# nelaturuharsha/TurboPrune

Measured on NVIDIA H100. Metric: images_per_sec_resnet50_erk80_train_step, higher is better.
Workload: dtype bf16

## Files before the change

### include/turboprune_b200.h

```cpp
#ifndef TURBOPRUNE_B200_H
#define TURBOPRUNE_B200_H

#include <stddef.h>
#include <stdint.h>

#ifdef __cplusplus
extern "C" {
#endif

#define TP_OK                 0
#define TP_ERR_INVALID       -1
#define TP_ERR_WORKSPACE     -2
#define TP_ERR_CUDA          -3
#define TP_ERR_K_RANGE       -4
#define TP_ERR_UNSUPPORTED   -5
#define TP_ERR_DEVICE        -6

const char* tp_strerror(int code);
const char* tp_last_cuda_error(void);
int         tp_abi_version(void);
int         tp_device_sm_count(void);
int         tp_set_pdl(int on);

#define TP_SCORE_MAG      0
#define TP_SCORE_SNIP     1
#define TP_SCORE_SYNFLOW  2

size_t tp_topk_workspace_bytes(int n_seg, int64_t total_numel);
int tp_topk_threshold_mask(const void* const* w, const void* const* g, const void* const* m,
                           void* const* mask_out, const int64_t* numel, int n_seg,
                           int64_t k, int score_kind, float* thr_out,
                           void* ws, size_t ws_bytes, int64_t* info_out, void* stream);
int tp_topk_enqueue(const void* const* w, const void* const* g, const void* const* m,
                    void* const* mask_out, const int64_t* numel, int n_seg,
                    int64_t k, int score_kind, float* thr_out,
                    void* ws, size_t ws_bytes, int table_cached, void* stream);
int tp_topk_finish(const void* const* m, void* const* mask_out, const int64_t* numel, int n_seg,
                   int64_t k, int score_kind, float* thr_out,
                   void* ws, size_t ws_bytes, int64_t* info_out, void* stream);

int tp_apply_threshold(const void* const* w, const void* const* g, const void* const* m,
                       void* const* mask_out, const int64_t* numel, int n_seg,
                       int score_kind, const float* thr, void* ws, size_t ws_bytes, void* stream);

int tp_count_zeros(const void* const* m, const int64_t* numel, int n_seg,
                   int64_t* zeros_out, void* ws, size_t ws_bytes, void* stream);

int tp_stage_weights(const void* w, const void* mask, int cout, int cin, int r, int s,
                     void* wf, int cin_p, int wf_ld, void* wd, int cout_p, int cin_p2,
                     void* kmask_f, void* kmask_d, void* stream);
size_t tp_kblock_mask_words(int64_t columns);

typedef struct tp_stage_item {
  const void* w; const void* mask;
  void* wf; void* wd;
  int32_t cout, cin, r, s, cin_p, cout_p, wf_ld;
  void* kmask_f; void* kmask_d;
} tp_stage_item;
size_t tp_stage_batched_workspace_bytes(int n_items);
int tp_stage_weights_batched(const tp_stage_item* items, int n_items, int table_cached, void* kmask_all, size_t kmask_bytes,
                             void* ws, size_t ws_bytes, void* stream);

int tp_to_nhwc_bf16(const void* src, int src_dtype, int64_t sn, int64_t sc, int64_t sh, int64_t sw,
                    int n, int c, int h, int w, void* dst, int c_pad, void* stream);

int tp_im2col_c8(const void* x, int n, int h, int w, int r, int s, int stride_h, int stride_w,
                 int pad_h, int pad_w, int p, int q, void* xcol, int kp, void* stream);

int tp_im2col_stem(const void* src, int src_dtype, int64_t sn, int64_t sc, int64_t sh, int64_t sw,
                   int n, int c, int h, int w, int r, int s, int cg, int stride_h, int stride_w, int pad_h, int pad_w,
                   int p, int q, void* xcol, int kp, void* stream);

int tp_cifar_augment(const void* src, void* out, const int64_t* idx, const int64_t* shifts, const uint8_t* flip,
                     const int64_t* cut_y, const int64_t* cut_x, int cut_size,
                     int n, int c, int h, int w, int r, void* stream);
typedef struct tp_crop_entry {
  const void* src;
  int32_t H, W;
  int32_t top, left, h, w;
  int32_t flip;
  int32_t reserved;
} tp_crop_entry;
int tp_resized_crop(const tp_crop_entry* table, int n, int size, const float* mean255, const float* std255, void* out,
                    void* stream);
int tp_synth_normal(void* out, int64_t numel, uint64_t seed, uint64_t counter_offset, int raw_words, void* stream);
int tp_synth_labels(void* out, int64_t numel, int num_classes, uint64_t seed, uint64_t counter_offset, void* stream);

typedef struct tp_conv_desc {
  int32_t n, h, w, cin;
  int32_t cout, r, s;
  int32_t stride_h, stride_w, pad_h, pad_w;
  int32_t p, q;
} tp_conv_desc;

size_t tp_conv_workspace_bytes(const tp_conv_desc* d, int op);

int tp_conv_fprop(const tp_conv_desc* d, const void* x, const void* wf, const void* bias_f32,
                  void* y, void* ws, size_t ws_bytes, void* stream);
size_t tp_conv_stats_rows(const tp_conv_desc* d);
int tp_conv_fprop_stats(const tp_conv_desc* d, const void* x, const void* wf, const void* kmask_f, const void* bias_f32,
                        void* y, void* stats, void* ws, size_t ws_bytes, void* stream);
int tp_conv_dgrad(const tp_conv_desc* d, const void* dy, const void* wd, const void* kmask_d, const void* addend,
                  void* dx, void* ws, size_t ws_bytes, void* stream);
size_t tp_conv_dgrad_partial_rows(const tp_conv_desc* d);
int tp_conv_dgrad_bnrelu(const tp_conv_desc* d, const void* dy, const void* wd, const void* kmask_d,
                         const void* bn_y, const void* bn_weight, const void* bn_bias, const void* bn_mean, const void* bn_invstd,
                         void* g, void* partial, void* stream);
int tp_conv_wgrad(const tp_conv_desc* d, const void* x, const void* dy, const void* mask, const void* kmask_f,
                  int cin_real, void* dw, void* db, void* ws, size_t ws_bytes, void* stream);

int tp_bn_forward_ext(const void* y, const void* residual, void* z, int64_t M, int C,
                      const void* weight, const void* bias, void* running_mean, void* running_var,
                      void* num_batches_tracked, float momentum, float eps, int training, int relu,
                      void* save_mean, void* save_invstd, const void* ext_stats, int64_t ext_rows,
                      void* ws, size_t ws_bytes, void* stream);

size_t tp_bn_workspace_bytes(int64_t m, int c);
int tp_bn_forward(const void* y, const void* residual, void* z, int64_t m, int c,
                  const void* weight, const void* bias, void* running_mean, void* running_var,
                  void* num_batches_tracked, float momentum, float eps, int training, int relu,
                  void* save_mean, void* save_invstd, void* ws, size_t ws_bytes, void* stream);
int tp_bn_backward(const void* dz, const void* z, const void* y, int64_t m, int c, const void* weight, const void* bias,
                   const void* save_mean, const void* save_invstd, int relu, void* dy, void* dres,
                   void* dweight, void* dbias, void* ws, size_t ws_bytes, void* stream);

int tp_bn_backward_ext(const void* g, const void* y, int64_t M, int C, const void* weight, const void* bias,
                       const void* save_mean, const void* save_invstd, const void* partial_rows, int64_t n_rows,
                       void* dy, void* dweight, void* dbias, void* ws, size_t ws_bytes, void* stream);
int tp_maxpool_forward(const void* x, void* y, void* idx, int n, int h, int w, int c, int k, int stride, int pad,
                       int p, int q, void* stream);
int tp_maxpool_backward(const void* dy, const void* idx, void* dx, int n, int h, int w, int c, int k, int stride, int pad,
                        int p, int q, void* stream);

int tp_sgd_momentum(void* const* w, const void* const* g, void* const* buf, const int64_t* numel,
                    int n_seg, const float* lr_dev, float momentum, float weight_decay,
                    int first_step, int table_cached, void* ws, size_t ws_bytes, void* stream);
size_t tp_segtable_workspace_bytes(int n_seg);

int tp_p2p_allreduce_mask(void* const* peer_bufs, void* const* signal_pads, int rank, int world,
                          int64_t numel, const void* mask, float scale, void* out,
                          int algo, int timeout_ms, int* status_dev, void* stream);

int tp_p2p_allreduce_nvls(void* const* peer_bufs, void* const* signal_pads, void* multicast_buf, int rank, int world,
                          int64_t numel, const void* mask, float scale, void* out,
                          int timeout_ms, int* status_dev, void* stream);

#ifdef __cplusplus
}
#endif
#endif
```

### turboprune_b200/_cabi.py

```python
import ctypes
import os
from ctypes import POINTER, c_char_p, c_float, c_int, c_int32, c_int64, c_size_t, c_uint64, c_void_p

from . import build as _build

TP_SCORE_MAG, TP_SCORE_SNIP, TP_SCORE_SYNFLOW = 0, 1, 2
TP_ERR_K_RANGE = -4

_lib = None


class ConvDesc(ctypes.Structure):
    _fields_ = [(n, c_int32) for n in
                ("n", "h", "w", "cin", "cout", "r", "s", "stride_h", "stride_w", "pad_h", "pad_w", "p", "q")]


class StageItem(ctypes.Structure):
    _fields_ = [("w", c_void_p), ("mask", c_void_p), ("wf", c_void_p), ("wd", c_void_p)] + \
               [(n, c_int32) for n in ("cout", "cin", "r", "s", "cin_p", "cout_p", "wf_ld")] + \
               [("kmask_f", c_void_p), ("kmask_d", c_void_p)]


class CropEntry(ctypes.Structure):
    _fields_ = [("src", c_void_p)] + [(n, c_int32) for n in ("H", "W", "top", "left", "h", "w", "flip", "reserved")]


SIGNATURES = {
    "tp_strerror": (c_char_p, [c_int]),
    "tp_last_cuda_error": (c_char_p, []),
    "tp_abi_version": (c_int, []),
    "tp_device_sm_count": (c_int, []),
    "tp_set_pdl": (c_int, [c_int]),
    "tp_topk_workspace_bytes": (c_size_t, [c_int, c_int64]),
    "tp_topk_threshold_mask": (c_int, [POINTER(c_void_p), POINTER(c_void_p), POINTER(c_void_p), POINTER(c_void_p),
                                       POINTER(c_int64), c_int, c_int64, c_int, c_void_p, c_void_p, c_size_t,
                                       POINTER(c_int64), c_void_p]),
    "tp_topk_enqueue": (c_int, [POINTER(c_void_p), POINTER(c_void_p), POINTER(c_void_p), POINTER(c_void_p),
                                POINTER(c_int64), c_int, c_int64, c_int, c_void_p, c_void_p, c_size_t, c_int, c_void_p]),
    "tp_topk_finish": (c_int, [POINTER(c_void_p), POINTER(c_void_p), POINTER(c_int64), c_int, c_int64, c_int, c_void_p,
                               c_void_p, c_size_t, POINTER(c_int64), c_void_p]),
    "tp_apply_threshold": (c_int, [POINTER(c_void_p), POINTER(c_void_p), POINTER(c_void_p), POINTER(c_void_p),
                                   POINTER(c_int64), c_int, c_int, c_void_p, c_void_p, c_size_t, c_void_p]),
    "tp_count_zeros": (c_int, [POINTER(c_void_p), POINTER(c_int64), c_int, c_void_p, c_void_p, c_size_t, c_void_p]),
    "tp_stage_weights": (c_int, [c_void_p, c_void_p, c_int, c_int, c_int, c_int, c_void_p, c_int, c_int, c_void_p, c_int,
                                 c_int, c_void_p, c_void_p, c_void_p]),
    "tp_kblock_mask_words": (c_size_t, [c_int64]),
    "tp_stage_batched_workspace_bytes": (c_size_t, [c_int]),
    "tp_stage_weights_batched": (c_int, [POINTER(StageItem), c_int, c_int, c_void_p, c_size_t, c_void_p, c_size_t, c_void_p]),
    "tp_to_nhwc_bf16": (c_int, [c_void_p, c_int, c_int64, c_int64, c_int64, c_int64, c_int, c_int, c_int, c_int,
                                c_void_p, c_int, c_void_p]),
    "tp_im2col_c8": (c_int, [c_void_p] + [c_int] * 11 + [c_void_p, c_int, c_void_p]),
    "tp_im2col_stem": (c_int, [c_void_p, c_int, c_int64, c_int64, c_int64, c_int64] + [c_int] * 13 + [c_void_p, c_int, c_void_p]),
    "tp_cifar_augment": (c_int, [c_void_p, c_void_p, c_void_p, c_void_p, c_void_p, c_void_p, c_void_p, c_int, c_int, c_int, c_int, c_int, c_int, c_void_p]),
    "tp_resized_crop": (c_int, [c_void_p, c_int, c_int, POINTER(c_float), POINTER(c_float), c_void_p, c_void_p]),
    "tp_synth_normal": (c_int, [c_void_p, c_int64, c_uint64, c_uint64, c_int, c_void_p]),
    "tp_synth_labels": (c_int, [c_void_p, c_int64, c_int, c_uint64, c_uint64, c_void_p]),
    "tp_conv_workspace_bytes": (c_size_t, [POINTER(ConvDesc), c_int]),
    "tp_conv_fprop": (c_int, [POINTER(ConvDesc), c_void_p, c_void_p, c_void_p, c_void_p, c_void_p, c_size_t, c_void_p]),
    "tp_conv_stats_rows": (c_size_t, [POINTER(ConvDesc)]),
    "tp_conv_fprop_stats": (c_int, [POINTER(ConvDesc), c_void_p, c_void_p, c_void_p, c_void_p, c_void_p, c_void_p, c_void_p, c_size_t, c_void_p]),
    "tp_conv_dgrad": (c_int, [POINTER(ConvDesc), c_void_p, c_void_p, c_void_p, c_void_p, c_void_p, c_void_p, c_size_t, c_void_p]),
    "tp_conv_dgrad_partial_rows": (c_size_t, [POINTER(ConvDesc)]),
    "tp_conv_dgrad_bnrelu": (c_int, [POINTER(ConvDesc), c_void_p, c_void_p, c_void_p, c_void_p, c_void_p, c_void_p, c_void_p, c_void_p,
                                     c_void_p, c_void_p, c_void_p]),
    "tp_bn_backward_ext": (c_int, [c_void_p, c_void_p, c_int64, c_int, c_void_p, c_void_p, c_void_p, c_void_p, c_void_p, c_int64,
                                   c_void_p, c_void_p, c_void_p, c_void_p, c_size_t, c_void_p]),
    "tp_conv_wgrad": (c_int, [POINTER(ConvDesc), c_void_p, c_void_p, c_void_p, c_void_p, c_int, c_void_p, c_void_p, c_void_p,
                              c_size_t, c_void_p]),
    "tp_sgd_momentum": (c_int, [POINTER(c_void_p), POINTER(c_void_p), POINTER(c_void_p), POINTER(c_int64), c_int,
                                c_void_p, c_float, c_float, c_int, c_int, c_void_p, c_size_t, c_void_p]),
    "tp_segtable_workspace_bytes": (c_size_t, [c_int]),
    "tp_p2p_allreduce_mask": (c_int, [POINTER(c_void_p), POINTER(c_void_p), c_int, c_int, c_int64, c_void_p, c_float,
                                      c_void_p, c_int, c_int, c_void_p, c_void_p]),
    "tp_bn_workspace_bytes": (c_size_t, [c_int64, c_int]),
    "tp_bn_forward": (c_int, [c_void_p, c_void_p, c_void_p, c_int64, c_int, c_void_p, c_void_p, c_void_p, c_void_p, c_void_p,
                              c_float, c_float, c_int, c_int, c_void_p, c_void_p, c_void_p, c_size_t, c_void_p]),
    "tp_bn_forward_ext": (c_int, [c_void_p, c_void_p, c_void_p, c_int64, c_int, c_void_p, c_void_p, c_void_p, c_void_p, c_void_p,
                                  c_float, c_float, c_int, c_int, c_void_p, c_void_p, c_void_p, c_int64, c_void_p, c_size_t, c_void_p]),
    "tp_bn_backward": (c_int, [c_void_p, c_void_p, c_void_p, c_int64, c_int, c_void_p, c_void_p, c_void_p, c_void_p, c_int, c_void_p,
                               c_void_p, c_void_p, c_void_p, c_void_p, c_size_t, c_void_p]),
    "tp_maxpool_forward": (c_int, [c_void_p, c_void_p, c_void_p] + [c_int] * 9 + [c_void_p]),
    "tp_maxpool_backward": (c_int, [c_void_p, c_void_p, c_void_p] + [c_int] * 9 + [c_void_p]),
    "tp_p2p_allreduce_nvls": (c_int, [POINTER(c_void_p), POINTER(c_void_p), c_void_p, c_int, c_int, c_int64, c_void_p, c_float,
                                      c_void_p, c_int, c_void_p, c_void_p]),
}


def lib_path() -> str:
    return _build.lib_path()


def load(build_if_missing: bool = False):
    global _lib
    if _lib is not None:
        return _lib
    path = lib_path()
    if not os.path.isfile(path):
        if build_if_missing:
            _build.build()
        else:
            raise RuntimeError(
                f"turboprune_b200: CUDA library not built ({path} missing). "
                "Run `python -c 'import __graft_entry__ as g; g.build()'`; there is no CPU fallback.")
    lib = ctypes.CDLL(path)
    for name, (res, args) in SIGNATURES.items():
        fn = getattr(lib, name)
        fn.restype = res
        fn.argtypes = args
    _lib = lib
    return lib


class TurboPruneError(RuntimeError):
    def __init__(self, code, where):
        lib = load()
        msg = lib.tp_strerror(code).decode()
        detail = lib.tp_last_cuda_error().decode() if code == -3 else ""
        super().__init__(f"{where}: {msg} (code {code}) {detail}".strip())
        self.code = code


def check(code: int, where: str):
    if code != 0:
        raise TurboPruneError(code, where)


def ptr_array(tensors):
    if tensors is None:
        return None
    arr = (c_void_p * len(tensors))()
    for i, t in enumerate(tensors):
        arr[i] = t.data_ptr() if t is not None else None
    return arr


def i64_array(vals):
    arr = (c_int64 * len(vals))()
    for i, v in enumerate(vals):
        arr[i] = int(v)
    return arr


def stream_ptr(device=None):
    import torch
    return c_void_p(torch.cuda.current_stream(device).cuda_stream)
```

### turboprune_b200/csrc/tp_common.cuh

```cuda
#pragma once
#include <cuda_runtime.h>
#include <cuda_bf16.h>
#include <stdint.h>
#include <stdio.h>
#include "../../include/turboprune_b200.h"

namespace tp {

void set_last_cuda_error(cudaError_t e, const char* where);

#define TP_CUDA_CHECK(expr)                                             \
  do {                                                                  \
    cudaError_t _e = (expr);                                            \
    if (_e != cudaSuccess) {                                            \
      ::tp::set_last_cuda_error(_e, #expr);                             \
      return TP_ERR_CUDA;                                               \
    }                                                                   \
  } while (0)

#define TP_LAUNCH_CHECK() TP_CUDA_CHECK(cudaGetLastError())

int sm_count();
int bind_device_of(const void* p);
inline size_t align_up(size_t x, size_t a) { return (x + a - 1) / a * a; }

bool pdl_enabled();
#ifdef __CUDACC__
__device__ __forceinline__ void pdl_wait() { asm volatile("griddepcontrol.wait;" ::: "memory"); }
__device__ __forceinline__ void pdl_trigger() { asm volatile("griddepcontrol.launch_dependents;" ::: "memory"); }
__device__ __forceinline__ void pdl_enter() { pdl_trigger(); pdl_wait(); }

template <typename... KA, typename... A>
inline cudaError_t launch(void (*kernel)(KA...), dim3 grid, dim3 block, size_t smem, cudaStream_t st, A&&... args) {
  cudaLaunchConfig_t cfg = {};
  cfg.gridDim = grid; cfg.blockDim = block; cfg.dynamicSmemBytes = smem; cfg.stream = st;
  cudaLaunchAttribute attr[1];
  attr[0].id = cudaLaunchAttributeProgrammaticStreamSerialization;
  attr[0].val.programmaticStreamSerializationAllowed = 1;
  cfg.attrs = attr; cfg.numAttrs = pdl_enabled() ? 1 : 0;
  return cudaLaunchKernelEx(&cfg, kernel, static_cast<KA>(args)...);
}
#endif

struct Arena {
  char* base; size_t cap; size_t off;
  Arena(void* p, size_t bytes) : base((char*)p), cap(bytes), off(0) {}
  void* take(size_t bytes, size_t align = 256) {
    size_t o = align_up(off, align);
    if (o + bytes > cap) return nullptr;
    off = o + bytes;
    return base + o;
  }
};

struct Seg {
  const float* w;
  const float* g;
  const float* m;
  float*       mo;
  float*       buf;
  long long    n;
  long long    start;
  long long    tile0;
};

constexpr int kTileElems = 4096;

int upload_segs(Arena& ar, const void* const* w, const void* const* g, const void* const* m,
                void* const* mo, void* const* buf, const int64_t* numel, int n_seg,
                Seg** dev_out, long long* tiles_out, long long* total_out, cudaStream_t st);

__device__ __forceinline__ int find_seg(const Seg* __restrict__ segs, int n_seg, long long tile) {
  int lo = 0, hi = n_seg - 1;
  while (lo < hi) {
    int mid = (lo + hi + 1) >> 1;
    if (segs[mid].tile0 <= tile) lo = mid; else hi = mid - 1;
  }
  return lo;
}
__device__ __forceinline__ int find_seg_by_elem(const Seg* __restrict__ segs, int n_seg, long long e) {
  int lo = 0, hi = n_seg - 1;
  while (lo < hi) {
    int mid = (lo + hi + 1) >> 1;
    if (segs[mid].start <= e) lo = mid; else hi = mid - 1;
  }
  return lo;
}

__device__ __forceinline__ float4 ld_stream(const float4* p) {
  float4 r;
  asm volatile("ld.global.nc.L1::no_allocate.v4.f32 {%0,%1,%2,%3}, [%4];"
               : "=f"(r.x), "=f"(r.y), "=f"(r.z), "=f"(r.w) : "l"(p));
  return r;
}
__device__ __forceinline__ void st_stream(float4* p, float4 v) {
  asm volatile("st.global.L1::no_allocate.v4.f32 [%0], {%1,%2,%3,%4};"
               :: "l"(p), "f"(v.x), "f"(v.y), "f"(v.z), "f"(v.w) : "memory");
}

}
```

### turboprune_b200/csrc/tp_core.cu

```cuda
#include "tp_common.cuh"
#include <stdlib.h>
#include <string.h>
#include <vector>

namespace tp {

static thread_local char g_last_err[512] = "";

void set_last_cuda_error(cudaError_t e, const char* where) {
  snprintf(g_last_err, sizeof(g_last_err), "%s: %s (%s)", where, cudaGetErrorName(e), cudaGetErrorString(e));
}

static int g_pdl = -1;
bool pdl_enabled() {
  if (g_pdl < 0) { const char* e = getenv("TP_PDL"); g_pdl = (e && e[0] == '1') ? 1 : 0; }
  return g_pdl == 1;
}

int sm_count() {
  static int cached[64] = {0};
  int dev = 0;
  if (cudaGetDevice(&dev) != cudaSuccess || dev < 0 || dev >= 64) return 132;
  if (cached[dev] == 0) {
    int n = 0;
    if (cudaDeviceGetAttribute(&n, cudaDevAttrMultiProcessorCount, dev) != cudaSuccess || n <= 0) n = 132;
    cached[dev] = n;
  }
  return cached[dev];
}

typedef int (*PFN_cuCtxGetCurrent)(void**);
static PFN_cuCtxGetCurrent g_ctx_get_current = nullptr;

int bind_device_of(const void* p) {
  if (!p) return TP_OK;
  static bool looked_up = false;
  if (!looked_up) {
    void* fn = nullptr; cudaDriverEntryPointQueryResult q;
    if (cudaGetDriverEntryPoint("cuCtxGetCurrent", &fn, cudaEnableDefault, &q) == cudaSuccess) g_ctx_get_current = (PFN_cuCtxGetCurrent)fn;
    looked_up = true;
  }
  if (g_ctx_get_current) {
    void* ctx = nullptr;
    if (g_ctx_get_current(&ctx) == 0 && ctx != nullptr) return TP_OK;
  }
  cudaPointerAttributes a;
  if (cudaPointerGetAttributes(&a, p) != cudaSuccess) { cudaGetLastError(); return TP_OK; }
  if (a.type == cudaMemoryTypeDevice || a.type == cudaMemoryTypeManaged) {
    TP_CUDA_CHECK(cudaSetDevice(a.device));
  }
  return TP_OK;
}

int upload_segs(Arena& ar, const void* const* w, const void* const* g, const void* const* m,
                void* const* mo, void* const* buf, const int64_t* numel, int n_seg,
                Seg** dev_out, long long* tiles_out, long long* total_out, cudaStream_t st) {
  if (n_seg <= 0 || !numel) return TP_ERR_INVALID;
  std::vector<Seg> h(n_seg);
  long long start = 0, tile = 0;
  for (int i = 0; i < n_seg; ++i) {
    if (numel[i] < 0) return TP_ERR_INVALID;
    h[i].w = w ? (const float*)w[i] : nullptr;
    h[i].g = g ? (const float*)g[i] : nullptr;
    h[i].m = m ? (const float*)m[i] : nullptr;
    h[i].mo = mo ? (float*)mo[i] : nullptr;
    h[i].buf = buf ? (float*)buf[i] : nullptr;
    h[i].n = numel[i];
    h[i].start = start;
    h[i].tile0 = tile;
    start += numel[i];
    tile += (numel[i] + kTileElems - 1) / kTileElems;
  }
  Seg* d = (Seg*)ar.take(sizeof(Seg) * n_seg);
  if (!d) return TP_ERR_WORKSPACE;
  TP_CUDA_CHECK(cudaMemcpyAsync(d, h.data(), sizeof(Seg) * n_seg, cudaMemcpyHostToDevice, st));
  *dev_out = d;
  if (tiles_out) *tiles_out = tile;
  if (total_out) *total_out = start;
  return TP_OK;
}

}

extern "C" {

const char* tp_strerror(int code) {
  switch (code) {
    case TP_OK: return "ok";
    case TP_ERR_INVALID: return "invalid argument";
    case TP_ERR_WORKSPACE: return "workspace too small";
    case TP_ERR_CUDA: return "CUDA error (see tp_last_cuda_error)";
    case TP_ERR_K_RANGE: return "kthvalue(): selected number k out of range";
    case TP_ERR_UNSUPPORTED: return "unsupported configuration";
    case TP_ERR_DEVICE: return "device is not sm_90 (H100)";
    default: return "unknown error";
  }
}

const char* tp_last_cuda_error(void) { return tp::g_last_err; }
int tp_abi_version(void) { return 10; }
int tp_device_sm_count(void) { return tp::sm_count(); }
int tp_set_pdl(int on) { const int prev = tp::pdl_enabled() ? 1 : 0; tp::g_pdl = on ? 1 : 0; return prev; }

size_t tp_segtable_workspace_bytes(int n_seg) {
  return tp::align_up(sizeof(tp::Seg) * (size_t)(n_seg > 0 ? n_seg : 1), 256) + 256;
}

}
```

### turboprune_b200/csrc/tp_igemm.cu

```cuda
#include "tp_common.cuh"
#include "tp_ptx.cuh"
#include <cuda.h>
#include <mutex>

namespace tp {
using namespace ptx;

constexpr int kBlockM = 128;
constexpr int kBlockK = 64;
constexpr int kConsumers = 256;
constexpr int kThreads = kConsumers + 32;
constexpr int kProducerWarp = kConsumers / 32;
constexpr int kFwdThreads = 3 * 128;
constexpr int kMaxTaps = 64;

constexpr int kFwdProducerRegs = 56, kFwdConsumerRegs = 224;
static_assert(kFwdProducerRegs * 128 + kFwdConsumerRegs * 256 <= 168 * kFwdThreads, "fwd register split");

__host__ __device__ constexpr int fwd_stages(int block_n) { return block_n == 128 ? 5 : 8; }
__host__ __device__ constexpr int fwd_stg_bytes(int block_n) { return kBlockM * block_n * 2; }
__host__ __device__ constexpr int fwd_smem(int block_n) {
  return fwd_stages(block_n) * (kBlockM * kBlockK * 2 + block_n * kBlockK * 2) + 2 * fwd_stg_bytes(block_n) + 1024 + 512;
}

struct TapEntry { uint16_t off_w, off_h; int32_t kofs; };

constexpr int kMaxCls = 4;

struct ClsEntry {
  int M;
  int P_it, Q_it;
  int ntaps, tap0;
  int base_w, base_h;
  int oah, oaw;
  int tile0, m_groups;
};

struct FwdParams {
  int M, N;
  int ncls;
  ClsEntry cls[kMaxCls];
  int cchunks;
  int a_mode;
  int step_w, step_h;
  long long out_img_pix;
  int out_row_pix;
  int osh, osw;
  int linear;
  int ldc;
  int staged_store;
  __nv_bfloat16* out;
  const float* bias;
  const __nv_bfloat16* addend;
  float* stats;
  const __nv_bfloat16* bn_y;
  const float* bn_weight; const float* bn_bias; const float* bn_mean; const float* bn_invstd;
  const uint32_t* kmask;
  int kmask_words;
  TapEntry taps[kMaxTaps];
};

__device__ __forceinline__ const uint32_t* live_kmask(const uint32_t* km, int words, int N) {
  if (km && __ldg(km + (size_t)((N + 63) >> 6) * words) == 0u) return nullptr;
  return km;
}

struct KSkip {
  const uint32_t* base; int words, g0, g1; int cur_w; uint32_t bits;
  __device__ __forceinline__ void begin(const uint32_t* km, int wds, int n0, int block_n, int N) {
    base = km; words = wds; cur_w = -1; bits = 0u;
    g0 = n0 >> 6; g1 = min((min(n0 + block_n, N) + 63) >> 6, ((N + 63) >> 6));
  }
  __device__ __forceinline__ bool on(int kb) {
    const int wi = kb >> 5;
    if (wi != cur_w) {
      cur_w = wi; bits = 0u;
      if (wi < words) for (int g = g0; g < g1; ++g) bits |= __ldg(base + (size_t)g * words + wi);
      else bits = 0xffffffffu;
    }
    return (bits >> (kb & 31)) & 1u;
  }
  __device__ __forceinline__ bool take(int kb, bool last, bool any) { return on(kb) || (last && !any); }
};

struct WgParams {
  int Mc;
  int Kpix;
  int P_it, Q_it;
  int chunks, cchunks;
  int nb;
  int b_mode;
  int base_w, base_h, step_w, step_h;
  int m_tiles, n_tiles, splits, kb_per_split, kblocks;
  float* partial;
  const uint32_t* kmask;
  int kmask_words;
  TapEntry taps[kMaxTaps];
};

struct WgItem {
  int split, tile, m_t, n_t, chunk0, nvalid, kb0, kb1;
  __device__ __forceinline__ void set_tile(int m, int n, int m_tiles, int nb, int chunks) {
    m_t = m; n_t = n; tile = n * m_tiles + m;
    chunk0 = n * nb; nvalid = min(nb, chunks - chunk0);
  }
  __device__ __forceinline__ bool empty(const uint32_t* __restrict__ km, int words, int Mc) const {
    const int row_groups = (Mc + 63) >> 6;
    for (int r = 2 * m_t; r < 2 * m_t + 2 && r < row_groups; ++r)
      for (int c = chunk0; c < chunk0 + nvalid; ++c)
        if ((__ldg(km + (size_t)r * words + (c >> 5)) >> (c & 31)) & 1u) return false;
    return true;
  }
};

__device__ __forceinline__ WgItem wg_item(const WgParams& p, int nb, int item) {
  WgItem w;
  const int ntile = p.m_tiles * p.n_tiles;
  w.split = item / ntile;
  const int tile = item - w.split * ntile, n_t = tile / p.m_tiles;
  w.set_tile(tile - n_t * p.m_tiles, n_t, p.m_tiles, nb, p.chunks);
  w.kb0 = w.split * p.kb_per_split; w.kb1 = min(p.kblocks, w.kb0 + p.kb_per_split);
  return w;
}

__device__ __forceinline__ void decompose_pixel(int m, int P, int Q, int& n, int& p, int& q) {
  q = m % Q; int t = m / Q; p = t % P; n = t / P;
}

struct AMaps { CUtensorMap m[kMaxCls]; };

__device__ __forceinline__ void decode_tile(const FwdParams& p, int tile, int n_tiles, int& c, int& m_g, int& n_t) {
  c = 0;
#pragma unroll
  for (int j = 1; j < kMaxCls; ++j) if (j < p.ncls && tile >= p.cls[j].tile0) c = j;
  const int local = tile - p.cls[c].tile0;
  m_g = local / n_tiles; n_t = local - m_g * n_tiles;
}

template <int BLOCK_N>
__device__ __forceinline__ void fwd_mma_block(float (&acc)[BLOCK_N], uint32_t a_addr, uint32_t b_addr, uint32_t accumulate) {
  const uint64_t adesc = make_smem_desc(a_addr, 16, 1024);
  const uint64_t adesc_hi = make_smem_desc(a_addr + 64 * kBlockK * 2, 16, 1024);
  const uint64_t bdesc = make_smem_desc(b_addr, 16, 1024);
#pragma unroll
  for (int k = 0; k < kBlockK / 16; ++k) {
    if constexpr (BLOCK_N == 128) {
      wgmma_m64n128<0, 0>(acc, adesc + (uint64_t)(2 * k), bdesc + (uint64_t)(2 * k), accumulate | (uint32_t)k);
      wgmma_m64n128<0, 0>(acc + BLOCK_N / 2, adesc_hi + (uint64_t)(2 * k), bdesc + (uint64_t)(2 * k), accumulate | (uint32_t)k);
    } else {
      wgmma_m64n64<0, 0>(acc, adesc + (uint64_t)(2 * k), bdesc + (uint64_t)(2 * k), accumulate | (uint32_t)k);
      wgmma_m64n64<0, 0>(acc + BLOCK_N / 2, adesc_hi + (uint64_t)(2 * k), bdesc + (uint64_t)(2 * k), accumulate | (uint32_t)k);
    }
  }
}

template <int BLOCK_N, bool MULTI, bool BNB>
__global__ void __launch_bounds__(kFwdThreads, 1)
k_igemm_fwd(const __grid_constant__ AMaps tmA, const __grid_constant__ CUtensorMap tmB,
            const __grid_constant__ FwdParams p) {
  static_assert(BLOCK_N == 64 || BLOCK_N == 128, "wgmma N of the fwd kernel");
  static_assert(!BNB || !MULTI, "BatchNorm-backward epilogue: single class");
  constexpr int kABytes = kBlockM * kBlockK * 2;
  constexpr int kBBytes = BLOCK_N * kBlockK * 2;
  constexpr int kStageBytes = kABytes + kBBytes;
  constexpr int kStages = fwd_stages(BLOCK_N);
  extern __shared__ __align__(1024) uint8_t smem_raw[];
  uint8_t* smem = (uint8_t*)(((uintptr_t)smem_raw + 1023) & ~(uintptr_t)1023);
  pdl_trigger();
  constexpr int kStgBytes = fwd_stg_bytes(BLOCK_N);
  constexpr int kChunkStg = kBlockM * 64 * 2;
  uint8_t* const stg_base = smem + kStages * kStageBytes;
  uint64_t* full_bar = (uint64_t*)(stg_base + 2 * kStgBytes);
  uint64_t* empty_bar = full_bar + kStages;
  uint64_t* order_bar = empty_bar + kStages;
  int* ring_pos = (int*)(order_bar + 2);

  const int warp = threadIdx.x >> 5, lane = threadIdx.x & 31;
  const int n_tiles = (p.N + BLOCK_N - 1) / BLOCK_N;
  const int total_tiles = p.cls[p.ncls - 1].tile0 + p.cls[p.ncls - 1].m_groups * n_tiles;
  const int my_items = total_tiles > (int)blockIdx.x ? (total_tiles - (int)blockIdx.x + (int)gridDim.x - 1) / (int)gridDim.x : 0;
  auto get_tile = [&](int w, int& ci, int& m_g, int& n_t) {
    ci = 0;
    const int tile = (int)blockIdx.x + w * (int)gridDim.x;
    if (MULTI) decode_tile(p, tile, n_tiles, ci, m_g, n_t);
    else { m_g = tile / n_tiles; n_t = tile - m_g * n_tiles; }
  };

  if (threadIdx.x == 0) {
    for (int j = 0; j < p.ncls; ++j) prefetch_tmap(&tmA.m[j]);
    prefetch_tmap(&tmB);
    for (int i = 0; i < kStages; ++i) { mbar_init(&full_bar[i], 1); mbar_init(&empty_bar[i], 1); }
    mbar_init(&order_bar[0], 1); mbar_init(&order_bar[1], 1);
    fence_mbar_init();
  }
  __syncthreads();
  pdl_wait();

  if (warp < 4) {
    setmaxnreg_dec<kFwdProducerRegs>();
    if (threadIdx.x == 0) {
      int stage = 0; uint32_t phase = 0;
      const uint32_t* const km = live_kmask(p.kmask, p.kmask_words, p.N);
      for (int w = 0; w < my_items; ++w) {
        int ci, m_g, n_t; get_tile(w, ci, m_g, n_t);
        const ClsEntry& ce = p.cls[MULTI ? ci : 0];
        const CUtensorMap* const mapA = &tmA.m[MULTI ? ci : 0];
        const int m0 = m_g * kBlockM;
        int cn = 0, cp = 0, cq = 0;
        if (p.a_mode == 1) decompose_pixel(m0, ce.P_it, ce.Q_it, cn, cp, cq);
        const int cw = ce.base_w + cq * p.step_w, ch = ce.base_h + cp * p.step_h;
        auto load_block = [&](const TapEntry& te, int cc) {
          mbar_wait(&empty_bar[stage], phase ^ 1);
          uint8_t* sA = smem + stage * kStageBytes;
          uint8_t* sB = sA + kABytes;
          mbar_arrive_expect_tx(&full_bar[stage], kStageBytes);
          if (p.a_mode == 1)
            tma_load_im2col_4d(sA, mapA, &full_bar[stage], cc * kBlockK, cw, ch, cn, te.off_w, te.off_h);
          else
            tma_load_2d(sA, mapA, &full_bar[stage], te.kofs + cc * kBlockK, m0);
          tma_load_2d(sB, &tmB, &full_bar[stage], te.kofs + cc * kBlockK, n_t * BLOCK_N);
          if (++stage == kStages) { stage = 0; phase ^= 1; }
        };
        const int tap_base = MULTI ? ce.tap0 : 0;
        if (!km) {
          for (int tap = 0; tap < ce.ntaps; ++tap) {
            const TapEntry te = p.taps[tap_base + tap];
            for (int cc = 0; cc < p.cchunks; ++cc) load_block(te, cc);
          }
        } else {
          KSkip ks; bool any = false;
          ks.begin(km, p.kmask_words, n_t * BLOCK_N, BLOCK_N, p.N);
          for (int tap = 0; tap < ce.ntaps; ++tap) {
            const TapEntry te = p.taps[tap_base + tap];
            for (int cc = 0; cc < p.cchunks; ++cc) {
              const bool last = tap == ce.ntaps - 1 && cc == p.cchunks - 1;
              if (!ks.take((te.kofs >> 6) + cc, last, any)) continue;
              any = true;
              load_block(te, cc);
            }
          }
        }
      }
    }
  } else {
    setmaxnreg_inc<kFwdConsumerRegs>();
    const int cw = (warp >> 2) - 1;
    const int q = warp & 3;
    const int wtid = threadIdx.x & 127;
    const int bar_id = 1 + cw;
    const uint32_t* const km = live_kmask(p.kmask, p.kmask_words, p.N);
    const uint32_t stg = smem_u32(stg_base + cw * kStgBytes);
    const int fr0 = q * 16 + (lane >> 2);
    const uint32_t fsw = (uint32_t)(lane >> 2);
    const uint32_t frag_base = stg + (uint32_t)(fr0 * 128 + (lane & 3) * 4);
    const int r_in = lane >> 3, c16 = lane & 7;
    const uint32_t buf = stg + (uint32_t)(q * 32 * 128);
    const uint32_t rd_even = buf + r_in * 128 + ((uint32_t)(c16 ^ r_in) << 4);
    const uint32_t rd_odd = buf + (r_in + 4) * 128 + ((uint32_t)(c16 ^ (r_in + 4)) << 4);
    for (int it = 0, w = cw; w < my_items; ++it, w += 2) {
      int ci, m_g, n_t; get_tile(w, ci, m_g, n_t);
      const ClsEntry& ce = p.cls[MULTI ? ci : 0];
      const bool has_acc = MULTI ? ce.ntaps > 0 : true;
      const int m_t = m_g;

      int stage = 0; uint32_t phase = 0;
      const int turn = it + cw;
      if (turn > 0) {
        mbar_wait(&order_bar[cw], (uint32_t)((turn - 1) & 1));
        const int pos = *(volatile int*)ring_pos;
        stage = pos >> 1; phase = (uint32_t)(pos & 1);
      }
      bar_sync(bar_id, 128);
      auto pass_turn = [&]() {
        if (wtid == 0) { *(volatile int*)ring_pos = stage * 2 + (int)phase; mbar_arrive(&order_bar[cw ^ 1]); }
      };
      float acc[BLOCK_N];
      if (has_acc) {
#pragma unroll
        for (int i = 0; i < BLOCK_N; ++i) acc[i] = 0.f;
        int prev = -1;
        auto mma_block = [&](uint32_t accumulate) {
          mbar_wait(&full_bar[stage], phase);
          const uint32_t s_addr = smem_u32(smem + stage * kStageBytes);
          wgmma_fence();
          fwd_mma_block<BLOCK_N>(acc, s_addr, s_addr + kABytes, accumulate);
          wgmma_commit();
          wgmma_wait<1>();
          if (prev >= 0 && wtid == 0) mbar_arrive(&empty_bar[prev]);
          prev = stage;
          if (++stage == kStages) { stage = 0; phase ^= 1; }
        };
        KSkip ks; uint32_t any = 0;
        if (km) ks.begin(km, p.kmask_words, n_t * BLOCK_N, BLOCK_N, p.N);
        for (int tap = 0; tap < ce.ntaps; ++tap) {
          const int kb0 = p.taps[(MULTI ? ce.tap0 : 0) + tap].kofs >> 6;
          for (int cc = 0; cc < p.cchunks; ++cc) {
            const bool last = tap == ce.ntaps - 1 && cc == p.cchunks - 1;
            if (km && !ks.take(kb0 + cc, last, any)) continue;
            mma_block(any);
            any = 1;
          }
        }
        pass_turn();
        wgmma_wait<0>();
        acc_fence(acc);
        if (prev >= 0 && wtid == 0) mbar_arrive(&empty_bar[prev]);
      } else {
        pass_turn();
      }

      const long long wrow0 = (long long)m_t * kBlockM + q * 32;
      const int rows_left = (int)(ce.M - wrow0 < 32 ? (ce.M - wrow0 < 0 ? 0 : ce.M - wrow0) : 32);
      const long long ldc = p.ldc;
      const int N = p.N;
      long long ooff[MULTI ? 8 : 1];
      const long long rbase = (wrow0 + r_in) * ldc + c16 * 8;
      if (MULTI && p.staged_store) {
        int n, pp, qq; decompose_pixel((int)(wrow0 + r_in), ce.P_it, ce.Q_it, n, pp, qq);
#pragma unroll
        for (int i = 0; i < 8; ++i) {
          const long long px = (long long)n * p.out_img_pix + (long long)(pp * p.osh + ce.oah) * p.out_row_pix + (qq * p.osw + ce.oaw);
          ooff[i] = px * ldc + c16 * 8;
          qq += 4;
          while (qq >= ce.Q_it) { qq -= ce.Q_it; if (++pp == ce.P_it) { pp = 0; ++n; } }
        }
      }
      auto row_off = [&](int i) -> long long { return MULTI ? ooff[MULTI ? i : 0] : rbase + (long long)(i * 4) * ldc; };
      if (MULTI && !has_acc) {
        if (p.staged_store) {
#pragma unroll 1
          for (int c = 0; c < BLOCK_N; c += 64) {
            const int n0 = n_t * BLOCK_N + c;
            if (n0 >= N) break;
            if (n0 + c16 * 8 + 8 > N) continue;
            uint4 z[8];
#pragma unroll
            for (int i = 0; i < 8; ++i) {
              z[i] = make_uint4(0u, 0u, 0u, 0u);
              if (p.addend && i * 4 + r_in < rows_left) z[i] = *reinterpret_cast<const uint4*>(p.addend + row_off(i) + n0);
            }
#pragma unroll
            for (int i = 0; i < 8; ++i)
              if (i * 4 + r_in < rows_left) *reinterpret_cast<uint4*>(p.out + row_off(i) + n0) = z[i];
          }
        } else {
          const int row = m_t * kBlockM + wtid;
          if (row < ce.M) {
            int n, pp, qq; decompose_pixel(row, ce.P_it, ce.Q_it, n, pp, qq);
            const long long opix = (long long)n * p.out_img_pix + (long long)(pp * p.osh + ce.oah) * p.out_row_pix + (qq * p.osw + ce.oaw);
            for (int j = n_t * BLOCK_N; j < min(p.N, (n_t + 1) * BLOCK_N); ++j)
              p.out[opix * p.ldc + j] = p.addend ? p.addend[opix * p.ldc + j] : __float2bfloat16_rn(0.f);
          }
        }
        continue;
      }
      if (p.staged_store) {
        __nv_bfloat16* const gout = p.out;
        const __nv_bfloat16* const gadd = p.addend;
        const float* bias = p.bias;
        float* stats = p.stats ? p.stats + (long long)(m_t * 4 + q) * 2 * N + c16 * 8 : nullptr;
        if (gadd) {
          __syncwarp();
#pragma unroll
          for (int ch = 0; ch < BLOCK_N / 64; ++ch) {
            const int n0 = n_t * BLOCK_N + ch * 64;
            if (n0 >= N) break;
            const bool col_ok = n0 + c16 * 8 + 8 <= N;
            uint4 a[8];
#pragma unroll
            for (int i = 0; i < 8; ++i) {
              a[i] = make_uint4(0u, 0u, 0u, 0u);
              if (i * 4 + r_in < rows_left && col_ok) a[i] = *reinterpret_cast<const uint4*>(gadd + row_off(i) + n0);
            }
#pragma unroll
            for (int i = 0; i < 8; ++i) sts128(((i & 1) ? rd_odd : rd_even) + (uint32_t)(ch * kChunkStg + (i >> 1) * 1024), a[i]);
          }
        }
        bar_sync(bar_id, 128);
#pragma unroll
        for (int ch = 0; ch < BLOCK_N / 64; ++ch) {
          const int n0 = n_t * BLOCK_N + ch * 64;
          if (n0 >= N) break;
#pragma unroll
          for (int mh = 0; mh < 2; ++mh)
#pragma unroll
            for (int h = 0; h < 2; ++h)
#pragma unroll
              for (int j = 0; j < 8; ++j) {
                const int i = mh * (BLOCK_N / 2) + 4 * (ch * 8 + j) + 2 * h;
                float f0 = acc[i], f1 = acc[i + 1];
                const int n = n0 + 8 * j + 2 * (lane & 3);
                if (bias) {
                  if (n < N) f0 += bias[n];
                  if (n + 1 < N) f1 += bias[n + 1];
                }
                const uint32_t addr = frag_base + (uint32_t)(ch * kChunkStg + (64 * mh + 8 * h) * 128) + (((uint32_t)j ^ fsw) << 4);
                if (gadd) {
                  const uint32_t a = lds32(addr);
                  const float2 t2 = __bfloat1622float2(*reinterpret_cast<const __nv_bfloat162*>(&a));
                  f0 += t2.x; f1 += t2.y;
                }
                const __nv_bfloat162 hv = __floats2bfloat162_rn(f0, f1);
                sts32(addr, *reinterpret_cast<const uint32_t*>(&hv));
              }
        }
        bar_sync(bar_id, 128);
#pragma unroll 1
        for (int ch = 0; ch < BLOCK_N / 64; ++ch) {
          const int n0 = n_t * BLOCK_N + ch * 64;
          if (n0 >= N) break;
          const bool col_ok = n0 + c16 * 8 + 8 <= N;
          uint4 o[8];
#pragma unroll
          for (int i = 0; i < 8; ++i) o[i] = lds128(((i & 1) ? rd_odd : rd_even) + (uint32_t)(ch * kChunkStg + (i >> 1) * 1024));
          float s1[8], s2[8];
#pragma unroll
          for (int qq = 0; qq < 8; ++qq) { s1[qq] = 0.f; s2[qq] = 0.f; }
          if (BNB) {
            uint4 yv[8];
#pragma unroll
            for (int i = 0; i < 8; ++i) {
              yv[i] = make_uint4(0u, 0u, 0u, 0u);
              if (i * 4 + r_in < rows_left && col_ok) yv[i] = *reinterpret_cast<const uint4*>(p.bn_y + row_off(i) + n0);
            }
            float sc[8], sf[8], is_[8], nm[8];
            if (col_ok) {
              const int cb = n0 + c16 * 8;
#pragma unroll
              for (int qq = 0; qq < 8; qq += 4) {
                const float4 one4 = make_float4(1.f, 1.f, 1.f, 1.f), zero4 = make_float4(0.f, 0.f, 0.f, 0.f);
                const float4 a4 = p.bn_weight ? *reinterpret_cast<const float4*>(p.bn_weight + cb + qq) : one4;
                const float4 b4 = p.bn_bias ? *reinterpret_cast<const float4*>(p.bn_bias + cb + qq) : zero4;
                const float4 m4 = *reinterpret_cast<const float4*>(p.bn_mean + cb + qq), i4 = *reinterpret_cast<const float4*>(p.bn_invstd + cb + qq);
                is_[qq] = i4.x; is_[qq + 1] = i4.y; is_[qq + 2] = i4.z; is_[qq + 3] = i4.w;
                nm[qq] = m4.x; nm[qq + 1] = m4.y; nm[qq + 2] = m4.z; nm[qq + 3] = m4.w;
                sc[qq] = a4.x * i4.x; sc[qq + 1] = a4.y * i4.y; sc[qq + 2] = a4.z * i4.z; sc[qq + 3] = a4.w * i4.w;
                sf[qq] = fmaf(-m4.x, sc[qq], b4.x); sf[qq + 1] = fmaf(-m4.y, sc[qq + 1], b4.y);
                sf[qq + 2] = fmaf(-m4.z, sc[qq + 2], b4.z); sf[qq + 3] = fmaf(-m4.w, sc[qq + 3], b4.w);
              }
            } else {
#pragma unroll
              for (int qq = 0; qq < 8; ++qq) { sc[qq] = 0.f; sf[qq] = 0.f; is_[qq] = 0.f; nm[qq] = 0.f; }
            }
#pragma unroll
            for (int i = 0; i < 8; ++i) {
              if (i * 4 + r_in < rows_left) {
                __nv_bfloat162* gh = reinterpret_cast<__nv_bfloat162*>(&o[i]);
                const __nv_bfloat162* yh = reinterpret_cast<const __nv_bfloat162*>(&yv[i]);
#pragma unroll
                for (int qq = 0; qq < 4; ++qq) {
                  float2 d2 = __bfloat1622float2(gh[qq]);
                  const float2 y2 = __bfloat1622float2(yh[qq]);
                  if (!(fmaf(y2.x, sc[2 * qq], sf[2 * qq]) > 0.f)) d2.x = 0.f;
                  if (!(fmaf(y2.y, sc[2 * qq + 1], sf[2 * qq + 1]) > 0.f)) d2.y = 0.f;
                  gh[qq] = __floats2bfloat162_rn(d2.x, d2.y);
                  s1[2 * qq] += d2.x;     s2[2 * qq] = fmaf(d2.x, (y2.x - nm[2 * qq]) * is_[2 * qq], s2[2 * qq]);
                  s1[2 * qq + 1] += d2.y; s2[2 * qq + 1] = fmaf(d2.y, (y2.y - nm[2 * qq + 1]) * is_[2 * qq + 1], s2[2 * qq + 1]);
                }
              }
            }
          }
#pragma unroll
          for (int i = 0; i < 8; ++i)
            if (i * 4 + r_in < rows_left && col_ok) *reinterpret_cast<uint4*>(gout + row_off(i) + n0) = o[i];
          if (!BNB && stats) {
#pragma unroll
            for (int i = 0; i < 8; ++i) {
              if (i * 4 + r_in < rows_left) {
                const __nv_bfloat162* h2 = reinterpret_cast<const __nv_bfloat162*>(&o[i]);
#pragma unroll
                for (int qq = 0; qq < 4; ++qq) {
                  const float2 t2 = __bfloat1622float2(h2[qq]);
                  s1[2 * qq] += t2.x; s2[2 * qq] = fmaf(t2.x, t2.x, s2[2 * qq]);
                  s1[2 * qq + 1] += t2.y; s2[2 * qq + 1] = fmaf(t2.y, t2.y, s2[2 * qq + 1]);
                }
              }
            }
          }
          if (BNB || stats) {
#pragma unroll
            for (int qq = 0; qq < 8; ++qq) {
              s1[qq] += __shfl_xor_sync(0xffffffffu, s1[qq], 8);  s2[qq] += __shfl_xor_sync(0xffffffffu, s2[qq], 8);
              s1[qq] += __shfl_xor_sync(0xffffffffu, s1[qq], 16); s2[qq] += __shfl_xor_sync(0xffffffffu, s2[qq], 16);
            }
            if (r_in == 0 && col_ok) {
              float4* d1 = reinterpret_cast<float4*>(stats + n0);
              float4* d2 = reinterpret_cast<float4*>(stats + N + n0);
              d1[0] = make_float4(s1[0], s1[1], s1[2], s1[3]); d1[1] = make_float4(s1[4], s1[5], s1[6], s1[7]);
              d2[0] = make_float4(s2[0], s2[1], s2[2], s2[3]); d2[1] = make_float4(s2[4], s2[5], s2[6], s2[7]);
            }
          }
        }
      } else {
#pragma unroll
        for (int mh = 0; mh < 2; ++mh)
#pragma unroll
          for (int h = 0; h < 2; ++h) {
            const int row = m_t * kBlockM + fr0 + 8 * h + 64 * mh;
            if (row >= ce.M) continue;
            long long opix = row;
            if (MULTI || !p.linear) {
              int n, pp, qq; decompose_pixel(row, ce.P_it, ce.Q_it, n, pp, qq);
              opix = (long long)n * p.out_img_pix + (long long)(pp * p.osh + ce.oah) * p.out_row_pix + (qq * p.osw + ce.oaw);
            }
            __nv_bfloat16* const orow = p.out + opix * p.ldc;
#pragma unroll
            for (int j = 0; j < BLOCK_N / 8; ++j)
#pragma unroll
              for (int e = 0; e < 2; ++e) {
                const int n = n_t * BLOCK_N + 8 * j + 2 * (lane & 3) + e;
                if (n >= N) continue;
                float f = acc[mh * (BLOCK_N / 2) + 4 * j + 2 * h + e];
                if (p.bias) f += p.bias[n];
                if (p.addend) f += __bfloat162float(p.addend[opix * p.ldc + n]);
                orow[n] = __float2bfloat16_rn(f);
              }
          }
      }
    }
  }
}

template <int NB>
__device__ __forceinline__ void wgrad_mma_block(float (&acc)[NB * 32], uint32_t a_addr, uint32_t b_addr, bool first) {
  constexpr uint32_t kChunk = 64 * kBlockK * 2;
#pragma unroll
  for (int k = 0; k < kBlockK / 16; ++k) {
    const uint32_t acc_on = (!first || k > 0) ? 1u : 0u;
    const uint64_t adesc = make_smem_desc(a_addr + (uint32_t)(2048 * k), kChunk, 1024);
    const uint32_t bk = b_addr + (uint32_t)(2048 * k);
    if constexpr (NB >= 2) wgmma_m64n128<1, 1>(acc, adesc, make_smem_desc(bk, kChunk, 1024), acc_on);
    else wgmma_m64n64<1, 1>(acc, adesc, make_smem_desc(bk, kChunk, 1024), acc_on);
    if constexpr (NB == 4) wgmma_m64n128<1, 1>(acc + 64, adesc, make_smem_desc(bk + 2 * kChunk, kChunk, 1024), acc_on);
    if constexpr (NB == 3) wgmma_m64n64<1, 1>(acc + 64, adesc, make_smem_desc(bk + 2 * kChunk, kChunk, 1024), acc_on);
  }
}

template <int NB>
__global__ void __launch_bounds__(kThreads, 1)
k_igemm_wgrad(const __grid_constant__ CUtensorMap tmA ,
              const __grid_constant__ CUtensorMap tmB ,
              const __grid_constant__ WgParams p) {
  constexpr int kABytes = kBlockM * kBlockK * 2;
  constexpr int kChunkBytes = 64 * kBlockK * 2;
  constexpr int kMaxNb = 4;
  constexpr int kStageBytes = kABytes + kMaxNb * kChunkBytes;
  constexpr int kStages = 4;
  pdl_trigger();
  extern __shared__ __align__(1024) uint8_t smem_raw[];
  uint8_t* smem = (uint8_t*)(((uintptr_t)smem_raw + 1023) & ~(uintptr_t)1023);
  uint64_t* full_bar = (uint64_t*)(smem + kStages * kStageBytes);
  uint64_t* empty_bar = full_bar + kStages;

  const int warp = threadIdx.x >> 5, lane = threadIdx.x & 31;
  const int items = p.m_tiles * p.n_tiles * p.splits;
  constexpr int ncols = NB * 64;

  if (threadIdx.x == 0) {
    prefetch_tmap(&tmA); prefetch_tmap(&tmB);
    for (int i = 0; i < kStages; ++i) { mbar_init(&full_bar[i], 1); mbar_init(&empty_bar[i], kConsumers / 128); }
    fence_mbar_init();
  }
  __syncthreads();
  pdl_wait();
  const uint32_t* const km = live_kmask(p.kmask, p.kmask_words, p.Mc);

  if (warp == kProducerWarp) {
    if (lane == 0) {
      int stage = 0; uint32_t phase = 0;
      for (int item = blockIdx.x; item < items; item += gridDim.x) {
        const WgItem it = wg_item(p, NB, item);
        if (km && it.empty(km, p.kmask_words, p.Mc)) continue;
        const int m_t = it.m_t, chunk0 = it.chunk0, nvalid = it.nvalid, kb0 = it.kb0, kb1 = it.kb1;
        int c_c[4]; uint16_t c_ow[4], c_oh[4];
#pragma unroll
        for (int j = 0; j < 4; ++j) {
          const int chunk = min(chunk0 + j, p.chunks - 1), tap = chunk / p.cchunks;
          c_c[j] = (chunk - tap * p.cchunks) * 64; c_ow[j] = p.taps[tap].off_w; c_oh[j] = p.taps[tap].off_h;
        }
        int cn, cp, cq; decompose_pixel(kb0 * kBlockK, p.P_it, p.Q_it, cn, cp, cq);
        const int sq = kBlockK % p.Q_it, t1 = kBlockK / p.Q_it, sp = t1 % p.P_it, sn = t1 / p.P_it;
        for (int kb = kb0; kb < kb1; ++kb) {
          const int pix0 = kb * kBlockK;
          mbar_wait(&empty_bar[stage], phase ^ 1);
          mbar_arrive_expect_tx(&full_bar[stage], kABytes + nvalid * kChunkBytes);
          uint8_t* sA = smem + stage * kStageBytes;
          uint8_t* sB = sA + kABytes;
          tma_load_2d(sA, &tmA, &full_bar[stage], m_t * kBlockM, pix0);
          tma_load_2d(sA + kChunkBytes, &tmA, &full_bar[stage], m_t * kBlockM + 64, pix0);
          if (p.b_mode == 1) {
            const int cw = p.base_w + cq * p.step_w, ch = p.base_h + cp * p.step_h;
#pragma unroll
            for (int j = 0; j < 4; ++j)
              if (j < nvalid)
                tma_load_im2col_4d(sB + j * kChunkBytes, &tmB, &full_bar[stage], c_c[j], cw, ch, cn, c_ow[j], c_oh[j]);
            cq += sq; if (cq >= p.Q_it) { cq -= p.Q_it; cp += 1; }
            cp += sp; if (cp >= p.P_it) { cp -= p.P_it; cn += 1; }
            cn += sn;
          } else {
#pragma unroll
            for (int j = 0; j < 4; ++j)
              if (j < nvalid) tma_load_2d(sB + j * kChunkBytes, &tmB, &full_bar[stage], (chunk0 + j) * 64, pix0);
          }
          if (++stage == kStages) { stage = 0; phase ^= 1; }
        }
      }
    }
  } else {
    const int wg = warp >> 2;
    int stage = 0; uint32_t phase = 0;
    for (int item = blockIdx.x; item < items; item += gridDim.x) {
      const WgItem it = wg_item(p, NB, item);
      if (km && it.empty(km, p.kmask_words, p.Mc)) continue;
      const int kb0 = it.kb0, kb1 = it.kb1;
      float acc[NB * 32];
#pragma unroll
      for (int i = 0; i < NB * 32; ++i) acc[i] = 0.f;
      int prev = -1;
      for (int kb = kb0; kb < kb1; ++kb) {
        mbar_wait(&full_bar[stage], phase);
        const uint32_t a_addr = smem_u32(smem + stage * kStageBytes);
        wgmma_fence();
        wgrad_mma_block<NB>(acc, a_addr + (uint32_t)(wg * kChunkBytes), a_addr + kABytes, kb == kb0);
        wgmma_commit();
        wgmma_wait<1>();
        if (prev >= 0 && (threadIdx.x & 127) == 0) mbar_arrive(&empty_bar[prev]);
        prev = stage;
        if (++stage == kStages) { stage = 0; phase ^= 1; }
      }
      wgmma_wait<0>();
      acc_fence(acc);
      if (prev >= 0 && (threadIdx.x & 127) == 0) mbar_arrive(&empty_bar[prev]);
      float* ptile = p.partial + ((long long)it.tile * p.splits + it.split) * kBlockM * ncols;
      const int r0 = wg * 64 + (warp & 3) * 16 + (lane >> 2);
#pragma unroll
      for (int j = 0; j < ncols / 8; ++j)
#pragma unroll
        for (int h = 0; h < 2; ++h)
          *reinterpret_cast<float2*>(ptile + (long long)(r0 + 8 * h) * ncols + 8 * j + 2 * (lane & 3)) =
              make_float2(acc[4 * j + 2 * h], acc[4 * j + 2 * h + 1]);
    }
  }
}

__global__ void __launch_bounds__(256) k_wgrad_finalize(const float* __restrict__ partial, const float* __restrict__ mask,
                                                        float* __restrict__ dw, int cout, int cin_real, int cin_p, int rs,
                                                        int nb, int m_tiles, int splits, int sl,
                                                        const uint32_t* __restrict__ kmask, int kmask_words) {
  pdl_enter();
  __shared__ float s_lane[256];
  const uint32_t* const km = live_kmask(kmask, kmask_words, cout);
  const int co = blockIdx.x;
  const int r = co % kBlockM;
  const int ktot = rs * cin_p;
  const int ncols = nb * 64;
  const int KT = 256 / sl;
  const int kl = threadIdx.x % KT, sj = threadIdx.x / KT;
  const int kk = blockIdx.y * KT + kl;
  const long long sstride = (long long)kBlockM * ncols;
  float a[8] = {0.f, 0.f, 0.f, 0.f, 0.f, 0.f, 0.f, 0.f};
  bool skipped = false;
  if (kk < ktot) {
    const int chunk = kk >> 6;
    WgItem it; it.set_tile(co / kBlockM, chunk / nb, m_tiles, nb, (ktot + 63) >> 6);
    skipped = km && it.empty(km, kmask_words, cout);
    if (!skipped) {
      const float* base = partial + (((long long)it.tile * splits) * kBlockM + r) * ncols + (chunk - it.chunk0) * 64 + (kk & 63);
      int sp = sj;
      for (; sp + 7 * sl < splits; sp += 8 * sl) {
        float v[8];
#pragma unroll
        for (int j = 0; j < 8; ++j) v[j] = __ldcs(base + (long long)(sp + j * sl) * sstride);
#pragma unroll
        for (int j = 0; j < 8; ++j) a[j] += v[j];
      }
      for (; sp < splits; sp += sl) a[0] += __ldcs(base + (long long)sp * sstride);
    }
  }
  s_lane[sj * KT + kl] = ((a[0] + a[1]) + (a[2] + a[3])) + ((a[4] + a[5]) + (a[6] + a[7]));
  __syncthreads();
  if (sj == 0 && kk < ktot) {
    float acc = 0.f;
    for (int j = 0; j < sl; ++j) acc += s_lane[j * KT + kl];
    const int tap = kk / cin_p, ci = kk - tap * cin_p;
    if (ci < cin_real) {
      const long long o = ((long long)co * cin_real + ci) * rs + tap;
      dw[o] = skipped ? 0.f : mask[o] * acc;
    }
  }
}

__global__ void __launch_bounds__(256) k_colsum_part(const __nv_bfloat16* __restrict__ dy, long long npix, int c, int ldc,
                                                     float* __restrict__ part) {
  pdl_enter();
  __shared__ float s_acc[256][9];
  const int tx = threadIdx.x, ty = threadIdx.y, TX = blockDim.x, TY = blockDim.y;
  const int cvec = blockIdx.y * TX + tx;
  const bool act = cvec * 8 < c;
  float a[8];
#pragma unroll
  for (int i = 0; i < 8; ++i) a[i] = 0.f;
  auto add8 = [&](const uint4& v) {
    const __nv_bfloat162* h = reinterpret_cast<const __nv_bfloat162*>(&v);
#pragma unroll
    for (int i = 0; i < 4; ++i) { const float2 f = __bfloat1622float2(h[i]); a[2 * i] += f.x; a[2 * i + 1] += f.y; }
  };
  if (act) {
    const long long stride = (long long)gridDim.x * TY;
    long long p = (long long)blockIdx.x * TY + ty;
    const __nv_bfloat16* src = dy + (size_t)cvec * 8;
    for (; p + 3 * stride < npix; p += 4 * stride) {
      uint4 v[4];
#pragma unroll
      for (int u = 0; u < 4; ++u) v[u] = *reinterpret_cast<const uint4*>(src + (size_t)(p + u * stride) * ldc);
#pragma unroll
      for (int u = 0; u < 4; ++u) add8(v[u]);
    }
    for (; p < npix; p += stride) add8(*reinterpret_cast<const uint4*>(src + (size_t)p * ldc));
  }
  const int tid = ty * TX + tx;
#pragma unroll
  for (int i = 0; i < 8; ++i) s_acc[tid][i] = a[i];
  __syncthreads();
  if (ty == 0 && act) {
    float r[8];
#pragma unroll
    for (int i = 0; i < 8; ++i) r[i] = 0.f;
    for (int j = 0; j < TY; ++j)
#pragma unroll
      for (int i = 0; i < 8; ++i) r[i] += s_acc[j * TX + tx][i];
#pragma unroll
    for (int i = 0; i < 8; ++i) part[(size_t)blockIdx.x * c + cvec * 8 + i] = r[i];
  }
}

__global__ void __launch_bounds__(256) k_colsum_fold(const float* __restrict__ part, int nparts, int c, float* __restrict__ db) {
  pdl_enter();
  const int ch = blockIdx.x * blockDim.x + threadIdx.x;
  if (ch >= c) return;
  float s0 = 0.f, s1 = 0.f, s2 = 0.f, s3 = 0.f;
  int j = 0;
  for (; j + 3 < nparts; j += 4) {
    s0 += part[(size_t)j * c + ch]; s1 += part[(size_t)(j + 1) * c + ch];
    s2 += part[(size_t)(j + 2) * c + ch]; s3 += part[(size_t)(j + 3) * c + ch];
  }
  for (; j < nparts; ++j) s0 += part[(size_t)j * c + ch];
  db[ch] = (s0 + s1) + (s2 + s3);
}

typedef CUresult (*PFN_encodeTiled)(CUtensorMap*, CUtensorMapDataType, cuuint32_t, void*, const cuuint64_t*, const cuuint64_t*,
                                    const cuuint32_t*, const cuuint32_t*, CUtensorMapInterleave, CUtensorMapSwizzle,
                                    CUtensorMapL2promotion, CUtensorMapFloatOOBfill);
typedef CUresult (*PFN_encodeIm2col)(CUtensorMap*, CUtensorMapDataType, cuuint32_t, void*, const cuuint64_t*, const cuuint64_t*,
                                     const int*, const int*, cuuint32_t, cuuint32_t, const cuuint32_t*, CUtensorMapInterleave,
                                     CUtensorMapSwizzle, CUtensorMapL2promotion, CUtensorMapFloatOOBfill);
static PFN_encodeTiled g_encodeTiled = nullptr;
static PFN_encodeIm2col g_encodeIm2col = nullptr;
static int g_driver_version = 0;

static int load_driver_fns() {
  static std::once_flag once;
  static int rc = TP_OK;
  std::call_once(once, []() {
    void* f1 = nullptr; void* f2 = nullptr;
    cudaDriverEntryPointQueryResult q;
    if (cudaGetDriverEntryPoint("cuTensorMapEncodeTiled", &f1, cudaEnableDefault, &q) != cudaSuccess || !f1 ||
        cudaGetDriverEntryPoint("cuTensorMapEncodeIm2col", &f2, cudaEnableDefault, &q) != cudaSuccess || !f2) {
      set_last_cuda_error(cudaErrorUnknown, "cudaGetDriverEntryPoint(cuTensorMapEncode*)");
      rc = TP_ERR_CUDA;
      return;
    }
    g_encodeTiled = (PFN_encodeTiled)f1;
    g_encodeIm2col = (PFN_encodeIm2col)f2;
    cudaDriverGetVersion(&g_driver_version);
  });
  return rc;
}

static int fail_cu(CUresult r, const char* what) {
  static thread_local char buf[128];
  snprintf(buf, sizeof(buf), "%s -> CUresult %d", what, (int)r);
  set_last_cuda_error(cudaErrorInvalidValue, buf);
  return TP_ERR_CUDA;
}

static int make_tiled_map(CUtensorMap* m, const void* ptr, uint64_t cols, uint64_t rows, uint64_t ld_elems, uint32_t box_rows) {
  cuuint64_t dims[2] = {cols, rows};
  cuuint64_t strides[1] = {ld_elems * 2};
  cuuint32_t box[2] = {64, box_rows};
  cuuint32_t es[2] = {1, 1};
  CUresult r = g_encodeTiled(m, CU_TENSOR_MAP_DATA_TYPE_BFLOAT16, 2, const_cast<void*>(ptr), dims, strides, box, es,
                             CU_TENSOR_MAP_INTERLEAVE_NONE, CU_TENSOR_MAP_SWIZZLE_128B,
                             CU_TENSOR_MAP_L2_PROMOTION_L2_256B, CU_TENSOR_MAP_FLOAT_OOB_FILL_NONE);
  if (r != CUDA_SUCCESS) return fail_cu(r, "cuTensorMapEncodeTiled");
  return TP_OK;
}

static int make_im2col_map(CUtensorMap* m, const void* ptr, int n, int h, int w, int c,
                           int base_w, int base_h, int step_w, int step_h, int P_it, int Q_it, uint32_t pixels) {
  cuuint64_t dims[4] = {(cuuint64_t)c, (cuuint64_t)w, (cuuint64_t)h, (cuuint64_t)n};
  cuuint64_t strides[3] = {(cuuint64_t)c * 2, (cuuint64_t)w * c * 2, (cuuint64_t)h * w * c * 2};
  int lower[2] = {base_w, base_h};
  int upper[2] = {(Q_it - 1) * step_w + 1 + base_w - w, (P_it - 1) * step_h + 1 + base_h - h};
  cuuint32_t es[4] = {1, (cuuint32_t)step_w, (cuuint32_t)step_h, 1};
  CUresult r = g_encodeIm2col(m, CU_TENSOR_MAP_DATA_TYPE_BFLOAT16, 4, const_cast<void*>(ptr), dims, strides, lower, upper,
                              64, pixels, es, CU_TENSOR_MAP_INTERLEAVE_NONE, CU_TENSOR_MAP_SWIZZLE_128B,
                              CU_TENSOR_MAP_L2_PROMOTION_L2_256B, CU_TENSOR_MAP_FLOAT_OOB_FILL_NONE);
  if (r != CUDA_SUCCESS) return fail_cu(r, "cuTensorMapEncodeIm2col");
  if (g_driver_version <= 13010 && (size_t)n * h * w * c * 2 < 131072)
    reinterpret_cast<uint64_t*>(m)[1] &= ~(1ull << 21);
  return TP_OK;
}

struct WgGeom {
  int chunks, nb, m_tiles, n_tiles, kblocks, smax;
  size_t partial_bytes(int splits) const { return (size_t)m_tiles * n_tiles * splits * kBlockM * nb * 64 * sizeof(float); }
};

static WgGeom wgrad_geom(const tp_conv_desc* d) {
  WgGeom g;
  g.chunks = (d->r * d->s * d->cin + 63) / 64;
  g.nb = g.chunks >= 4 ? 4 : g.chunks;
  g.m_tiles = (d->cout + kBlockM - 1) / kBlockM;
  g.n_tiles = (g.chunks + g.nb - 1) / g.nb;
  g.kblocks = (int)(((long long)d->n * d->p * d->q + 63) / 64);
  g.smax = (2 * sm_count()) / (g.m_tiles * g.n_tiles);
  if (g.smax > g.kblocks) g.smax = g.kblocks;
  if (g.smax < 1) g.smax = 1;
  return g;
}

static int pick_wgrad_splits(const WgGeom& g) {
  const int sms = sm_count();
  const int tiles = g.m_tiles * g.n_tiles, kblocks = g.kblocks, nb = g.nb;
  const double c_kb = 0.30;
  const double c_part = 0.33 * nb;
  const double c_fin = 0.013 * nb;
  int best = 1; double best_cost = 1e30;
  for (int s = 1; s <= g.smax; ++s) {
    const int kb = (kblocks + s - 1) / s;
    const int s_eff = (kblocks + kb - 1) / kb;
    const long long items = (long long)tiles * s_eff;
    const long long waves = (items + sms - 1) / sms;
    const double cost = (double)waves * (kb * c_kb + c_part) + (double)items * c_fin;
    if (cost < best_cost - 1e-9) { best_cost = cost; best = s_eff; }
  }
  return best;
}

static bool is_plain_gemm(const tp_conv_desc* d) {
  return d->r == 1 && d->s == 1 && d->stride_h == 1 && d->stride_w == 1 && d->pad_h == 0 && d->pad_w == 0;
}

static void fill_taps(TapEntry* taps, int R, int S, int cin) {
  for (int r = 0; r < R; ++r) for (int s = 0; s < S; ++s) {
    TapEntry& t = taps[r * S + s];
    t.off_w = (uint16_t)s; t.off_h = (uint16_t)r; t.kofs = (r * S + s) * cin;
  }
}

static int pick_block_n(long long m_tiles, int n) {
  const int sms = sm_count();
  int best = 64; double best_score = -1;
  const int cands[2] = {128, 64};
  const double weight[2] = {1.0, 0.82};
  for (int i = 0; i < 2; ++i) {
    int bn = cands[i];
    if (bn > 64 && n <= bn / 2) continue;
    long long tiles = m_tiles * ((n + bn - 1) / bn);
    long long waves = (tiles + sms - 1) / sms;
    double eff = (double)tiles / (double)(waves * sms) * weight[i];
    if (eff > best_score) { best_score = eff; best = bn; }
  }
  return best;
}

constexpr int kSmemMax = 232448;

template <int BN, bool MULTI, bool BNB = false>
static int launch_fwd(const AMaps& a, const CUtensorMap& b, FwdParams& p, cudaStream_t st) {
  constexpr int smem = fwd_smem(BN);
  static_assert(smem <= kSmemMax, "fwd smem budget");
  const int n_tiles = (p.N + BN - 1) / BN;
  static bool attr_set = false;
  if (!attr_set) {
    TP_CUDA_CHECK(cudaFuncSetAttribute(k_igemm_fwd<BN, MULTI, BNB>, cudaFuncAttributeMaxDynamicSharedMemorySize, smem));
    attr_set = true;
  }
  long long ctiles = 0;
  for (int c = 0; c < p.ncls; ++c) {
    p.cls[c].m_groups = (int)((p.cls[c].M + kBlockM - 1) / kBlockM);
    if (ctiles > 0x7fffffffll) return TP_ERR_UNSUPPORTED;
    p.cls[c].tile0 = (int)ctiles;
    ctiles += (long long)p.cls[c].m_groups * n_tiles;
  }
  if (ctiles > 0x7fffffffll || ctiles <= 0) return TP_ERR_UNSUPPORTED;
  const int grid = (int)(ctiles < sm_count() ? ctiles : sm_count());
  TP_CUDA_CHECK(launch(k_igemm_fwd<BN, MULTI, BNB>, dim3(grid), dim3(kFwdThreads), (size_t)smem, st, a, b, p));
  TP_LAUNCH_CHECK();
  return TP_OK;
}

static int run_fwd(const AMaps& a, const CUtensorMap& b, FwdParams& p, int bn, cudaStream_t st) {
  p.linear = p.ncls == 1 && p.osh == 1 && p.osw == 1 && p.cls[0].oah == 0 && p.cls[0].oaw == 0 &&
             p.out_row_pix == p.cls[0].Q_it && p.out_img_pix == (long long)p.cls[0].P_it * p.cls[0].Q_it;
  p.staged_store = (p.ldc % 8 == 0 && p.N % 8 == 0 && (((uintptr_t)p.out) & 15) == 0 &&
                    (!p.addend || (((uintptr_t)p.addend) & 15) == 0)) ? 1 : 0;
  if (p.stats && !(p.staged_store && p.linear)) return TP_ERR_UNSUPPORTED;
  const bool multi = !p.linear;
  if (multi) {
    if (bn == 128) return launch_fwd<128, true>(a, b, p, st);
    return launch_fwd<64, true>(a, b, p, st);
  }
  if (p.bn_y) {
    if (!p.staged_store || !p.stats) return TP_ERR_UNSUPPORTED;
    if (bn == 128) return launch_fwd<128, false, true>(a, b, p, st);
    return launch_fwd<64, false, true>(a, b, p, st);
  }
  if (bn == 128) return launch_fwd<128, false>(a, b, p, st);
  return launch_fwd<64, false>(a, b, p, st);
}

template <int NB>
static int launch_wgrad(int grid, const CUtensorMap& ta, const CUtensorMap& tb, const WgParams& p, cudaStream_t st) {
  constexpr int smem = 4 * (kBlockM * kBlockK * 2 + 4 * 64 * kBlockK * 2) + 1024 + 256;
  static bool attr_set = false;
  if (!attr_set) {
    TP_CUDA_CHECK(cudaFuncSetAttribute(k_igemm_wgrad<NB>, cudaFuncAttributeMaxDynamicSharedMemorySize, smem));
    attr_set = true;
  }
  TP_CUDA_CHECK(launch(k_igemm_wgrad<NB>, dim3(grid), dim3(kThreads), (size_t)smem, st, ta, tb, p));
  TP_LAUNCH_CHECK();
  return TP_OK;
}

}

using namespace tp;

extern "C" {

size_t tp_conv_workspace_bytes(const tp_conv_desc* d, int op) {
  if (!d) return 0;
  if (op != 2) return 256;
  const WgGeom g = wgrad_geom(d);
  return g.partial_bytes(g.smax) + 1024;
}

size_t tp_conv_stats_rows(const tp_conv_desc* d) {
  if (!d) return 0;
  const long long M = (long long)d->n * d->p * d->q;
  return (size_t)((M + kBlockM - 1) / kBlockM) * 4;
}

int tp_conv_fprop(const tp_conv_desc* d, const void* x, const void* wf, const void* bias_f32,
                  void* y, void* ws, size_t ws_bytes, void* stream) {
  return tp_conv_fprop_stats(d, x, wf, nullptr, bias_f32, y, nullptr, ws, ws_bytes, stream);
}

int tp_conv_fprop_stats(const tp_conv_desc* d, const void* x, const void* wf, const void* kmask_f, const void* bias_f32,
                        void* y, void* stats, void* ws, size_t ws_bytes, void* stream) {
  (void)ws; (void)ws_bytes;
  if (!d || !x || !wf || !y) return TP_ERR_INVALID;
  if (stats && (d->cout % 8 != 0 || (((uintptr_t)y) & 15) != 0 || (((uintptr_t)stats) & 15) != 0)) return TP_ERR_UNSUPPORTED;
  if (d->cin % 8 != 0 || d->r * d->s > kMaxTaps) return TP_ERR_UNSUPPORTED;
  if (d->r * d->s > 1 && d->cin % 64 != 0) return TP_ERR_UNSUPPORTED;
  int rc = load_driver_fns(); if (rc) return rc;
  rc = bind_device_of(d ? (const void*)x : nullptr); if (rc) return rc;
  cudaStream_t st = (cudaStream_t)stream;
  FwdParams p = {};
  p.M = d->n * d->p * d->q; p.N = d->cout;
  p.ncls = 1;
  ClsEntry& ce = p.cls[0];
  ce.M = p.M; ce.P_it = d->p; ce.Q_it = d->q; ce.ntaps = d->r * d->s; ce.tap0 = 0; ce.oah = 0; ce.oaw = 0;
  p.cchunks = (d->cin + 63) / 64;
  p.out_img_pix = (long long)d->p * d->q; p.out_row_pix = d->q;
  p.osh = 1; p.osw = 1;
  p.ldc = d->cout; p.out = (__nv_bfloat16*)y; p.bias = (const float*)bias_f32;
  p.stats = (float*)stats;
  p.kmask = (const uint32_t*)kmask_f; p.kmask_words = (int)tp_kblock_mask_words((int64_t)d->r * d->s * d->cin);
  fill_taps(p.taps, d->r, d->s, d->cin);
  AMaps ta; CUtensorMap tb;
  if (is_plain_gemm(d)) {
    p.a_mode = 0;
    rc = make_tiled_map(&ta.m[0], x, (uint64_t)d->cin, (uint64_t)p.M, (uint64_t)d->cin, kBlockM); if (rc) return rc;
  } else {
    p.a_mode = 1;
    ce.base_w = -d->pad_w; ce.base_h = -d->pad_h; p.step_w = d->stride_w; p.step_h = d->stride_h;
    rc = make_im2col_map(&ta.m[0], x, d->n, d->h, d->w, d->cin, ce.base_w, ce.base_h, p.step_w, p.step_h, d->p, d->q, kBlockM);
    if (rc) return rc;
  }
  for (int c = 1; c < kMaxCls; ++c) ta.m[c] = ta.m[0];
  const int bn = pick_block_n((p.M + kBlockM - 1) / kBlockM, p.N);
  rc = make_tiled_map(&tb, wf, (uint64_t)d->r * d->s * d->cin, (uint64_t)d->cout, (uint64_t)d->r * d->s * d->cin, (uint32_t)bn);
  if (rc) return rc;
  return run_fwd(ta, tb, p, bn, st);
}

struct BnGate { const void* y; const float* weight; const float* bias; const float* mean; const float* invstd; float* partial; };

static int conv_dgrad_impl(const tp_conv_desc* d, const void* dy, const void* wd, const void* kmask_d, const void* addend,
                           void* dx, const BnGate* gate, void* stream);

int tp_conv_dgrad(const tp_conv_desc* d, const void* dy, const void* wd, const void* kmask_d, const void* addend,
                  void* dx, void* ws, size_t ws_bytes, void* stream) {
  (void)ws; (void)ws_bytes;
  return conv_dgrad_impl(d, dy, wd, kmask_d, addend, dx, nullptr, stream);
}

int tp_conv_dgrad_bnrelu(const tp_conv_desc* d, const void* dy, const void* wd, const void* kmask_d,
                         const void* bn_y, const void* bn_weight, const void* bn_bias, const void* bn_mean, const void* bn_invstd,
                         void* g, void* partial, void* stream) {
  if (!d || !bn_y || !bn_mean || !bn_invstd || !partial) return TP_ERR_INVALID;
  if (d->stride_h != 1 || d->stride_w != 1 || d->cin % 8 != 0) return TP_ERR_UNSUPPORTED;
  if ((((uintptr_t)bn_y) | ((uintptr_t)bn_weight) | ((uintptr_t)bn_bias) | ((uintptr_t)bn_mean) | ((uintptr_t)bn_invstd) | ((uintptr_t)partial)) & 15)
    return TP_ERR_UNSUPPORTED;
  BnGate bn = {bn_y, (const float*)bn_weight, (const float*)bn_bias, (const float*)bn_mean, (const float*)bn_invstd, (float*)partial};
  return conv_dgrad_impl(d, dy, wd, kmask_d, nullptr, g, &bn, stream);
}

size_t tp_conv_dgrad_partial_rows(const tp_conv_desc* d) {
  if (!d) return 0;
  const long long M = (long long)d->n * d->h * d->w;
  return (size_t)((M + kBlockM - 1) / kBlockM) * 4;
}

static int conv_dgrad_impl(const tp_conv_desc* d, const void* dy, const void* wd, const void* kmask_d, const void* addend,
                           void* dx, const BnGate* gate, void* stream) {
  if (!d || !dy || !wd || !dx) return TP_ERR_INVALID;
  const int cop = d->cout;
  if (cop % 8 != 0 || d->r * d->s > kMaxTaps) return TP_ERR_UNSUPPORTED;
  if (d->r * d->s > 1 && cop % 64 != 0) return TP_ERR_UNSUPPORTED;
  int rc = load_driver_fns(); if (rc) return rc;
  rc = bind_device_of(d ? (const void*)dy : nullptr); if (rc) return rc;
  cudaStream_t st = (cudaStream_t)stream;
  const int R = d->r, S = d->s;
  const long long ktot = (long long)R * S * cop;
  const int sh = d->stride_h, sw = d->stride_w;
  FwdParams p = {};
  p.N = d->cin;
  p.cchunks = (cop + 63) / 64;
  p.out_img_pix = (long long)d->h * d->w; p.out_row_pix = d->w;
  p.ldc = d->cin; p.out = (__nv_bfloat16*)dx; p.bias = nullptr; p.addend = (const __nv_bfloat16*)addend;
  p.kmask = (const uint32_t*)kmask_d; p.kmask_words = (int)tp_kblock_mask_words(ktot);
  p.step_w = 1; p.step_h = 1;
  if (gate) {
    p.bn_y = (const __nv_bfloat16*)gate->y; p.bn_weight = gate->weight; p.bn_bias = gate->bias; p.bn_mean = gate->mean; p.bn_invstd = gate->invstd;
    p.stats = gate->partial;
  }
  AMaps ta; CUtensorMap tb;
  if (sh == 1 && sw == 1) {
    p.M = d->n * d->h * d->w;
    p.ncls = 1; p.osh = 1; p.osw = 1;
    ClsEntry& ce = p.cls[0];
    ce.M = p.M; ce.P_it = d->h; ce.Q_it = d->w; ce.ntaps = R * S; ce.tap0 = 0; ce.oah = 0; ce.oaw = 0;
    fill_taps(p.taps, R, S, cop);
    if (is_plain_gemm(d)) {
      p.a_mode = 0;
      rc = make_tiled_map(&ta.m[0], dy, (uint64_t)cop, (uint64_t)p.M, (uint64_t)cop, kBlockM); if (rc) return rc;
    } else {
      p.a_mode = 1;
      ce.base_w = -(S - 1 - d->pad_w); ce.base_h = -(R - 1 - d->pad_h);
      rc = make_im2col_map(&ta.m[0], dy, d->n, d->p, d->q, cop, ce.base_w, ce.base_h, 1, 1, d->h, d->w, kBlockM);
      if (rc) return rc;
    }
    for (int c = 1; c < kMaxCls; ++c) ta.m[c] = ta.m[0];
  } else {
    if (sh * sw > kMaxCls || R * S > kMaxTaps) return TP_ERR_UNSUPPORTED;
    p.a_mode = 1; p.osh = sh; p.osw = sw;
    int nc = 0, nt = 0; long long Mtot = 0;
    for (int a = 0; a < sh; ++a) for (int b = 0; b < sw; ++b) {
      const int Hc = (d->h - a + sh - 1) / sh, Wc = (d->w - b + sw - 1) / sw;
      if (Hc <= 0 || Wc <= 0) continue;
      ClsEntry& ce = p.cls[nc];
      ce.M = d->n * Hc * Wc; ce.P_it = Hc; ce.Q_it = Wc; ce.oah = a; ce.oaw = b; ce.tap0 = nt; ce.ntaps = 0;
      int dh_min = 1 << 30, dw_min = 1 << 30;
      for (int r = 0; r < R; ++r) if ((a + d->pad_h - r) % sh == 0) dh_min = min(dh_min, (a + d->pad_h - r) / sh);
      for (int s = 0; s < S; ++s) if ((b + d->pad_w - s) % sw == 0) dw_min = min(dw_min, (b + d->pad_w - s) / sw);
      if (dh_min != (1 << 30) && dw_min != (1 << 30)) {
        for (int r = 0; r < R; ++r) {
          if ((a + d->pad_h - r) % sh != 0) continue;
          for (int s = 0; s < S; ++s) {
            if ((b + d->pad_w - s) % sw != 0) continue;
            TapEntry& t = p.taps[nt++];
            t.off_h = (uint16_t)((a + d->pad_h - r) / sh - dh_min);
            t.off_w = (uint16_t)((b + d->pad_w - s) / sw - dw_min);
            t.kofs = ((R - 1 - r) * S + (S - 1 - s)) * cop;
            ++ce.ntaps;
          }
        }
      } else { dh_min = 0; dw_min = 0; }
      ce.base_w = dw_min; ce.base_h = dh_min;
      rc = make_im2col_map(&ta.m[nc], dy, d->n, d->p, d->q, cop, ce.base_w, ce.base_h, 1, 1, Hc, Wc, kBlockM); if (rc) return rc;
      Mtot += ce.M; ++nc;
    }
    if (nc == 0) return TP_OK;
    for (int c = nc; c < kMaxCls; ++c) ta.m[c] = ta.m[0];
    p.ncls = nc; p.M = (int)Mtot;
  }
  long long m_tiles = 0;
  for (int c = 0; c < p.ncls; ++c) m_tiles += (p.cls[c].M + kBlockM - 1) / kBlockM;
  const int bn = pick_block_n(m_tiles, p.N);
  rc = make_tiled_map(&tb, wd, (uint64_t)ktot, (uint64_t)d->cin, (uint64_t)ktot, (uint32_t)bn); if (rc) return rc;
  return run_fwd(ta, tb, p, bn, st);
}

int tp_conv_wgrad(const tp_conv_desc* d, const void* x, const void* dy, const void* mask, const void* kmask_f,
                  int cin_real, void* dw, void* db, void* ws, size_t ws_bytes, void* stream) {
  if (!d || !x || !dy || !mask || !dw || !ws) return TP_ERR_INVALID;
  if (d->cin % 8 != 0 || d->cout % 8 != 0 || d->r * d->s > kMaxTaps || cin_real > d->cin) return TP_ERR_UNSUPPORTED;
  if (d->r * d->s > 1 && d->cin % 64 != 0) return TP_ERR_UNSUPPORTED;
  int rc = load_driver_fns(); if (rc) return rc;
  rc = bind_device_of(d ? (const void*)x : nullptr); if (rc) return rc;
  cudaStream_t st = (cudaStream_t)stream;
  const int rs = d->r * d->s;
  WgParams p = {};
  p.Mc = d->cout;
  p.Kpix = d->n * d->p * d->q;
  p.P_it = d->p; p.Q_it = d->q;
  const WgGeom g = wgrad_geom(d);
  p.chunks = g.chunks;
  p.cchunks = (d->cin + 63) / 64;
  p.nb = g.nb;
  p.m_tiles = g.m_tiles;
  p.n_tiles = g.n_tiles;
  p.kblocks = g.kblocks;
  const int sms = sm_count();
  int splits = pick_wgrad_splits(g);
  p.kb_per_split = (p.kblocks + splits - 1) / splits;
  splits = (p.kblocks + p.kb_per_split - 1) / p.kb_per_split;
  p.splits = splits;
  if (ws_bytes < g.partial_bytes(splits)) return TP_ERR_WORKSPACE;
  p.partial = (float*)ws;
  p.kmask = (const uint32_t*)kmask_f; p.kmask_words = (int)tp_kblock_mask_words((int64_t)rs * d->cin);
  fill_taps(p.taps, d->r, d->s, d->cin);
  CUtensorMap ta, tb;
  rc = make_tiled_map(&ta, dy, (uint64_t)d->cout, (uint64_t)p.Kpix, (uint64_t)d->cout, 64); if (rc) return rc;
  if (is_plain_gemm(d)) {
    p.b_mode = 0;
    rc = make_tiled_map(&tb, x, (uint64_t)d->cin, (uint64_t)p.Kpix, (uint64_t)d->cin, 64); if (rc) return rc;
  } else {
    p.b_mode = 1;
    p.base_w = -d->pad_w; p.base_h = -d->pad_h; p.step_w = d->stride_w; p.step_h = d->stride_h;
    rc = make_im2col_map(&tb, x, d->n, d->h, d->w, d->cin, p.base_w, p.base_h, p.step_w, p.step_h, d->p, d->q, 64);
    if (rc) return rc;
  }
  const int items = p.m_tiles * p.n_tiles * splits;
  const int grid = items < sms ? items : sms;
  switch (p.nb) {
    case 1: rc = launch_wgrad<1>(grid, ta, tb, p, st); break;
    case 2: rc = launch_wgrad<2>(grid, ta, tb, p, st); break;
    case 3: rc = launch_wgrad<3>(grid, ta, tb, p, st); break;
    default: rc = launch_wgrad<4>(grid, ta, tb, p, st); break;
  }
  if (rc) return rc;
  const int sl = splits >= 64 ? 8 : (splits >= 32 ? 4 : (splits >= 16 ? 2 : 1));
  const int fin_kt = 256 / sl;
  launch(k_wgrad_finalize, dim3(d->cout, (rs * d->cin + fin_kt - 1) / fin_kt), 256, 0, st,
      p.partial, (const float*)mask, (float*)dw, d->cout, cin_real, d->cin, rs, p.nb, p.m_tiles, splits, sl,
      p.kmask, p.kmask_words);
  TP_LAUNCH_CHECK();
  if (db) {
    const int c = d->cout, cv = c / 8;
    int tx = 1;
    while (tx < cv && tx < 256) tx <<= 1;
    const int ty = 256 / tx, ctiles = (cv + tx - 1) / tx;
    long long gx = ((long long)p.Kpix + (long long)ty * 4 - 1) / ((long long)ty * 4);
    const long long want = (long long)sms * 4 / ctiles, fit = (long long)(ws_bytes / ((size_t)c * sizeof(float)));
    if (gx > want) gx = want;
    if (gx > fit) gx = fit;
    if (gx < 1) gx = 1;
    if ((((uintptr_t)dy) & 15) != 0) return TP_ERR_INVALID;
    launch(k_colsum_part, dim3((unsigned)gx, (unsigned)ctiles), dim3(tx, ty), 0, st, (const __nv_bfloat16*)dy, (long long)p.Kpix, c, c, (float*)ws);
    launch(k_colsum_fold, (c + 255) / 256, 256, 0, st, (const float*)ws, (int)gx, c, (float*)db);
    TP_LAUNCH_CHECK();
  }
  return TP_OK;
}

}
```

### turboprune_b200/csrc/tp_optim.cu

```cuda
#include "tp_common.cuh"
#include <vector>

namespace tp {

constexpr int kCoT = 8;
constexpr int kSlabFloats = 8192;

__device__ __forceinline__ void stage_slab(const float* __restrict__ w, const float* __restrict__ mask, int co0, int cout,
                                           int c0, int c1, int cin, int rs, __nv_bfloat16* __restrict__ wf, int cin_p, int wf_ld,
                                           __nv_bfloat16* __restrict__ wd, int cout_p, bool zero_pad, float* s_slab,
                                           uint32_t* __restrict__ kmf, int kmf_words, uint32_t* __restrict__ kmd, int kmd_words) {
  const int t = threadIdx.x;
  const int cw = c1 - c0;
  const int per_co = cw * rs;
  const int nco = min(kCoT, cout - co0);
  for (int i = t; i < nco * per_co; i += blockDim.x) {
    const int cl = i / per_co, j = i - cl * per_co;
    const long long gi = ((long long)(co0 + cl) * cin + c0) * rs + j;
    const float mk = mask[gi], prod = mk * w[gi];
    s_slab[i] = prod;
    if (kmf && prod == 0.f && mk != 0.f) {
      const int c = j / rs, tap = j - c * rs, kb = (tap * cin_p + c0 + c) >> 6;
      atomicOr(&kmf[(size_t)(co0 >> 6) * kmf_words + (kb >> 5)], 1u << (kb & 31));
    }
  }
  __syncthreads();
  for (int i = t; i < nco * per_co; i += blockDim.x) {
    const int cl = i / per_co, j = i - cl * per_co;
    const int tap = j / cw, c = j - tap * cw;
    wf[(long long)(co0 + cl) * wf_ld + tap * cin_p + c0 + c] = __float2bfloat16_rn(s_slab[cl * per_co + c * rs + tap]);
  }
  if (wd) {
    for (int j = t; j < per_co; j += blockDim.x) {
      const int c = j / rs, tap = j - c * rs;
      float f[kCoT];
#pragma unroll
      for (int cl = 0; cl < kCoT; ++cl) f[cl] = cl < nco ? s_slab[cl * per_co + j] : 0.f;
      __nv_bfloat16* dst = wd + ((long long)(c0 + c) * rs + (rs - 1 - tap)) * cout_p + co0;
      if (co0 + kCoT <= cout_p) {
        uint4 v;
        __nv_bfloat162* hv = reinterpret_cast<__nv_bfloat162*>(&v);
#pragma unroll
        for (int q = 0; q < 4; ++q) hv[q] = __floats2bfloat162_rn(f[2 * q], f[2 * q + 1]);
        *reinterpret_cast<uint4*>(dst) = v;
      } else {
        for (int cl = 0; cl < kCoT && co0 + cl < cout_p; ++cl) dst[cl] = __float2bfloat16_rn(f[cl]);
      }
    }
  }
  if (kmf || (kmd && wd)) {
    const int warp = t >> 5, lane = t & 31, nwarps = blockDim.x >> 5;
    if (kmf) {
      for (int tap = 0; tap < rs; ++tap) {
        const int col0 = tap * cin_p + c0, col1 = tap * cin_p + c1;
        for (int kb = (col0 >> 6) + warp; kb <= ((col1 - 1) >> 6); kb += nwarps) {
          const int a = max(col0, kb << 6), b = min(col1, (kb + 1) << 6), wdt = b - a;
          bool nz = false;
          for (int e = lane; e < nco * wdt; e += 32) {
            const int cl = e / wdt, c = a + (e - cl * wdt) - tap * cin_p - c0;
            nz |= s_slab[cl * per_co + c * rs + tap] != 0.f;
          }
          if (__any_sync(0xffffffffu, nz) && lane == 0) atomicOr(&kmf[(size_t)(co0 >> 6) * kmf_words + (kb >> 5)], 1u << (kb & 31));
        }
      }
    }
    if (kmd && wd) {
      const int g0 = c0 >> 6, g1 = (c1 - 1) >> 6;
      for (int item = warp; item < rs * (g1 - g0 + 1); item += nwarps) {
        const int tap = item / (g1 - g0 + 1), g = g0 + item % (g1 - g0 + 1);
        const int a = max(c0, g << 6), b = min(c1, (g + 1) << 6), wdt = b - a;
        bool nz = false;
        for (int e = lane; e < nco * wdt; e += 32) {
          const int cl = e / wdt, c = a + (e - cl * wdt) - c0;
          nz |= s_slab[cl * per_co + c * rs + tap] != 0.f;
        }
        const int kb = ((rs - 1 - tap) * cout_p + co0) >> 6;
        if (__any_sync(0xffffffffu, nz) && lane == 0) atomicOr(&kmd[(size_t)g * kmd_words + (kb >> 5)], 1u << (kb & 31));
      }
    }
  }
  if (zero_pad && c0 == 0 && cin_p > cin) {
    const int padw = cin_p - cin;
    for (int i = t; i < nco * padw * rs; i += blockDim.x) {
      const int cl = i / (padw * rs), j = i - cl * (padw * rs);
      const int tap = j / padw, c = j - tap * padw;
      wf[(long long)(co0 + cl) * wf_ld + tap * cin_p + cin + c] = __float2bfloat16_rn(0.f);
    }
  }
}

__global__ void __launch_bounds__(256) k_stage_weights(const float* __restrict__ w, const float* __restrict__ mask,
                                                       int cout, int cin, int rs,
                                                       __nv_bfloat16* __restrict__ wf, int cin_p,
                                                       __nv_bfloat16* __restrict__ wd, int cout_p, int wf_ld,
                                                       uint32_t* __restrict__ kmf, int kmf_words,
                                                       uint32_t* __restrict__ kmd, int kmd_words) {
  pdl_enter();
  extern __shared__ float s_slab[];
  const int CC = (cin + gridDim.y - 1) / gridDim.y;
  const int c0 = blockIdx.y * CC;
  const int c1 = min(cin, c0 + CC);
  if (c0 >= c1) return;
  stage_slab(w, mask, blockIdx.x * kCoT, cout, c0, c1, cin, rs, wf, cin_p, wf_ld, wd, cout_p, true, s_slab, kmf, kmf_words, kmd, kmd_words);
}

struct StageItem {
  const float* w; const float* mask; __nv_bfloat16* wf; __nv_bfloat16* wd;
  int cout, cin, rs, cin_p, cout_p, ysplit, cc, wf_ld;
  long long cta0;
  uint32_t* kmf; uint32_t* kmd;
  int kmf_words, kmd_words;
};

__global__ void __launch_bounds__(256) k_stage_weights_batched(const StageItem* __restrict__ items, int n_items) {
  pdl_enter();
  extern __shared__ float s_slab[];
  int lo = 0, hi = n_items - 1;
  const long long b = blockIdx.x;
  while (lo < hi) {
    const int mid = (lo + hi + 1) >> 1;
    if (items[mid].cta0 <= b) lo = mid; else hi = mid - 1;
  }
  const StageItem it = items[lo];
  const int local = (int)(b - it.cta0);
  const int ct = local / it.ysplit, y = local - ct * it.ysplit;
  const int c0 = y * it.cc, c1 = min(it.cin, c0 + it.cc);
  if (ct * kCoT >= it.cout || c0 >= c1) return;
  stage_slab(it.w, it.mask, ct * kCoT, it.cout, c0, c1, it.cin, it.rs, it.wf, it.cin_p, it.wf_ld, it.wd, it.cout_p, false, s_slab,
             it.kmf, it.kmf_words, it.kmd, it.kmd_words);
}

__device__ __forceinline__ void kmask_count_empty(uint32_t* km, int rows, int words, int kblocks) {
  __shared__ unsigned int s_n;
  if (threadIdx.x == 0) s_n = 0;
  __syncthreads();
  unsigned int n = 0;
  for (int i = threadIdx.x; i < rows * words; i += blockDim.x) {
    const int wi = i % words;
    const int valid = min(32, kblocks - wi * 32);
    const uint32_t vm = valid >= 32 ? 0xffffffffu : ((1u << valid) - 1u);
    n += __popc(~km[i] & vm);
  }
  if (n) atomicAdd(&s_n, n);
  __syncthreads();
  if (threadIdx.x == 0) km[(size_t)rows * words] = s_n;
  __syncthreads();
}

__global__ void __launch_bounds__(256) k_kmask_summary(const StageItem* __restrict__ items, int n_items) {
  pdl_enter();
  const StageItem it = items[blockIdx.x];
  if (it.kmf) kmask_count_empty(it.kmf, (it.cout + 63) / 64, it.kmf_words, (it.wf_ld + 63) / 64);
  if (it.kmd && it.wd) kmask_count_empty(it.kmd, (it.cin + 63) / 64, it.kmd_words, (it.rs * it.cout_p + 63) / 64);
}

__global__ void __launch_bounds__(256) k_kmask_summary1(uint32_t* kmf, int rows_f, int words_f, int kb_f,
                                                         uint32_t* kmd, int rows_d, int words_d, int kb_d) {
  pdl_enter();
  if (kmf) kmask_count_empty(kmf, rows_f, words_f, kb_f);
  if (kmd) kmask_count_empty(kmd, rows_d, words_d, kb_d);
}

__global__ void k_zero_bf16(__nv_bfloat16* p, long long n) {
  pdl_enter();
  long long i = blockIdx.x * (long long)blockDim.x + threadIdx.x;
  long long stride = (long long)gridDim.x * blockDim.x;
  for (; i < n; i += stride) p[i] = __float2bfloat16_rn(0.f);
}

template <typename T>
__global__ void __launch_bounds__(256) k_to_nhwc(const T* __restrict__ src, long long sn, long long sc, long long sh, long long sw,
                                                 int n, int c, int h, int w, __nv_bfloat16* __restrict__ dst, int c_pad) {
  pdl_enter();
  long long total = (long long)n * h * w * c_pad;
  long long i = blockIdx.x * (long long)blockDim.x + threadIdx.x;
  long long stride = (long long)gridDim.x * blockDim.x;
  for (; i < total; i += stride) {
    int ci = (int)(i % c_pad);
    long long pix = i / c_pad;
    int wi = (int)(pix % w);
    long long t2 = pix / w;
    int hi = (int)(t2 % h);
    int ni = (int)(t2 / h);
    float v = 0.f;
    if (ci < c) v = (float)src[ni * sn + ci * sc + hi * sh + wi * sw];
    dst[i] = __float2bfloat16_rn(v);
  }
}


__global__ void __launch_bounds__(256) k_im2col_c8(const uint4* __restrict__ x, int n, int h, int w,
                                                   int R, int S, int stride_h, int stride_w, int pad_h, int pad_w,
                                                   int P, int Q, uint4* __restrict__ xcol, int kp8) {
  pdl_enter();
  const long long total = (long long)n * P * Q * kp8;
  long long i = blockIdx.x * (long long)blockDim.x + threadIdx.x;
  const long long step = (long long)gridDim.x * blockDim.x;
  for (; i < total; i += step) {
    const int cell = (int)(i % kp8);
    const long long pix = i / kp8;
    uint4 v = make_uint4(0u, 0u, 0u, 0u);
    if (cell < R * S) {
      const int r = cell / S, s = cell - r * S;
      const int q = (int)(pix % Q); const long long t2 = pix / Q;
      const int pp = (int)(t2 % P); const int ni = (int)(t2 / P);
      const int hi = pp * stride_h - pad_h + r, wi = q * stride_w - pad_w + s;
      if (hi >= 0 && hi < h && wi >= 0 && wi < w) v = x[((long long)ni * h + hi) * w + wi];
    }
    xcol[i] = v;
  }
}

template <typename T>
__global__ void __launch_bounds__(256) k_im2col_stem(const T* __restrict__ src, long long sn, long long sc, long long sh, long long sw,
                                                     int n, int c, int h, int w, int R, int S, int cg, int stride_h, int stride_w,
                                                     int pad_h, int pad_w, int P, int Q, uint4* __restrict__ xcol, int kp8) {
  pdl_enter();
  extern __shared__ uint32_t s_col[];
  const int kp = kp8 * 8;
  for (int e = threadIdx.x; e < kp; e += blockDim.x) {
    uint32_t v = 0xFFFFFFFFu;
    const int tap = e / cg, ch = e - tap * cg;
    if (tap < R * S && ch < c) { const int r = tap / S, s_ = tap - r * S; v = ((uint32_t)r << 16) | ((uint32_t)s_ << 8) | (uint32_t)ch; }
    s_col[e] = v;
  }
  __syncthreads();
  const long long total = (long long)n * P * Q * kp8;
  long long i = blockIdx.x * (long long)blockDim.x + threadIdx.x;
  const long long step = (long long)gridDim.x * blockDim.x;
  for (; i < total; i += step) {
    const int cell = (int)(i % kp8);
    const long long pix = i / kp8;
    const int q = (int)(pix % Q); const long long t2 = pix / Q;
    const int pp = (int)(t2 % P); const int ni = (int)(t2 / P);
    const int h0 = pp * stride_h - pad_h, w0 = q * stride_w - pad_w;
    const T* base = src + ni * sn;
    float f[8];
#pragma unroll
    for (int j = 0; j < 8; ++j) {
      const uint32_t cd = s_col[cell * 8 + j];
      const int hi = h0 + (int)(cd >> 16), wi = w0 + (int)((cd >> 8) & 0xFF);
      f[j] = 0.f;
      if (cd != 0xFFFFFFFFu && hi >= 0 && hi < h && wi >= 0 && wi < w) f[j] = (float)base[hi * sh + wi * sw + (long long)(cd & 0xFF) * sc];
    }
    uint4 v;
    __nv_bfloat162* hv = reinterpret_cast<__nv_bfloat162*>(&v);
#pragma unroll
    for (int j = 0; j < 4; ++j) hv[j] = __floats2bfloat162_rn(f[2 * j], f[2 * j + 1]);
    xcol[i] = v;
  }
}

template <typename T>
__global__ void __launch_bounds__(256) k_im2col_stem_rows(const T* __restrict__ src, long long sn, long long sc, long long sh, long long sw,
                                                          int n, int c, int h, int w, int R, int S, int cg, int stride_h, int stride_w,
                                                          int pad_h, int pad_w, int P, int Q, int QS, uint4* __restrict__ xcol, int kp8) {
  pdl_enter();
  extern __shared__ __align__(16) unsigned short s_patch[];
  const int pw = (QS - 1) * stride_w + S;
  const int pitch = pw * c;
  const int zero_slot = R * pitch;
  const int strips_q = (Q + QS - 1) / QS;
  const long long n_strips = (long long)n * P * strips_q;
  const int cells_per_pass = blockDim.x / kp8 * kp8 > 0 ? blockDim.x / kp8 : 0;
  const int cell = threadIdx.x % kp8, plane = threadIdx.x / kp8;
  const bool worker = plane < cells_per_pass;
  int off[8];
#pragma unroll
  for (int j = 0; j < 8; ++j) {
    const int e = cell * 8 + j, tap = e / cg, ch = e - tap * cg;
    off[j] = zero_slot;
    if (tap < R * S && ch < c) { const int r = tap / S, s_ = tap - r * S; off[j] = r * pitch + s_ * c + ch; }
  }
  for (long long strip = blockIdx.x; strip < n_strips; strip += gridDim.x) {
    const int sq = (int)(strip % strips_q); long long t = strip / strips_q;
    const int pp = (int)(t % P); const int ni = (int)(t / P);
    const int q0 = sq * QS, nq = min(QS, Q - q0);
    const int h0 = pp * stride_h - pad_h, w0 = q0 * stride_w - pad_w;
    __syncthreads();
    const T* base = src + ni * sn;
    const float inv_c = 1.0f / (float)c;
    for (int r = 0; r < R; ++r) {
      const int hh = h0 + r;
      const bool row_in = hh >= 0 && hh < h;
      const T* rowp = base + hh * sh;
      for (int rem = threadIdx.x; rem < pitch; rem += blockDim.x) {
        const int wi = (int)(((float)rem + 0.5f) * inv_c), ch = rem - wi * c;
        const int ww = w0 + wi;
        float v = 0.f;
        if (row_in && ww >= 0 && ww < w) v = (float)rowp[ww * sw + (long long)ch * sc];
        s_patch[r * pitch + rem] = __bfloat16_as_ushort(__float2bfloat16_rn(v));
      }
    }
    if (threadIdx.x == 0) s_patch[zero_slot] = 0;
    __syncthreads();
    if (worker) {
      const long long row0 = ((long long)ni * P + pp) * Q + q0;
      for (int ql = plane; ql < nq; ql += cells_per_pass) {
        const int qo = ql * stride_w * c;
        unsigned short hv[8];
#pragma unroll
        for (int j = 0; j < 8; ++j) hv[j] = s_patch[off[j] == zero_slot ? zero_slot : off[j] + qo];
        uint4 v;
        v.x = hv[0] | ((unsigned)hv[1] << 16); v.y = hv[2] | ((unsigned)hv[3] << 16);
        v.z = hv[4] | ((unsigned)hv[5] << 16); v.w = hv[6] | ((unsigned)hv[7] << 16);
        xcol[(row0 + ql) * kp8 + cell] = v;
      }
    }
  }
}

__global__ void __launch_bounds__(256) k_sgd(const Seg* __restrict__ segs, int n_seg, long long tiles,
                                             const float* __restrict__ lr_p, float mu, float wd, int first) {
  pdl_enter();
  const float lr = *lr_p;
  const int t = threadIdx.x;
  for (long long tile = blockIdx.x; tile < tiles; tile += gridDim.x) {
    const int si = find_seg(segs, n_seg, tile);
    const Seg sg = segs[si];
    const long long base = (tile - sg.tile0) * kTileElems;
    const long long rem = sg.n - base;
    const int n_in = rem < kTileElems ? (int)rem : kTileElems;
    float* wp = const_cast<float*>(sg.w) + base;
    const float* gp = sg.g + base;
    float* bp = sg.buf + base;
    bool vec = n_in == kTileElems && ((((uintptr_t)wp) | ((uintptr_t)gp) | ((uintptr_t)bp)) & 15) == 0;
    if (vec) {
#pragma unroll
      for (int it = 0; it < kTileElems / (256 * 4); ++it) {
        int q = it * 256 + t;
        float4 w = ((const float4*)wp)[q];
        float4 g = ld_stream((const float4*)gp + q);
        float4 b = first ? make_float4(0.f, 0.f, 0.f, 0.f) : ((const float4*)bp)[q];
        float4 d;
        d.x = fmaf(wd, w.x, g.x); d.y = fmaf(wd, w.y, g.y); d.z = fmaf(wd, w.z, g.z); d.w = fmaf(wd, w.w, g.w);
        if (!first) { b.x = __fadd_rn(__fmul_rn(mu, b.x), d.x); b.y = __fadd_rn(__fmul_rn(mu, b.y), d.y); b.z = __fadd_rn(__fmul_rn(mu, b.z), d.z); b.w = __fadd_rn(__fmul_rn(mu, b.w), d.w); }
        else b = d;
        w.x = fmaf(-lr, b.x, w.x); w.y = fmaf(-lr, b.y, w.y); w.z = fmaf(-lr, b.z, w.z); w.w = fmaf(-lr, b.w, w.w);
        ((float4*)bp)[q] = b;
        ((float4*)wp)[q] = w;
      }
    } else {
      for (int i = t; i < n_in; i += 256) {
        float w = wp[i], g = gp[i];
        float d = fmaf(wd, w, g);
        float b = first ? d : __fadd_rn(__fmul_rn(mu, bp[i]), d);
        bp[i] = b;
        wp[i] = fmaf(-lr, b, w);
      }
    }
  }
}

}

using namespace tp;

extern "C" {

size_t tp_kblock_mask_words(int64_t columns) {
  if (columns <= 0) return 0;
  return (size_t)(((columns + 63) / 64 + 31) / 32);
}

int tp_stage_weights(const void* w, const void* mask, int cout, int cin, int r, int s,
                     void* wf, int cin_p, int wf_ld, void* wd, int cout_p, int cin_p2,
                     void* kmask_f, void* kmask_d, void* stream) {
  if (!w || !mask || !wf || cout <= 0 || cin <= 0 || r <= 0 || s <= 0 || cin_p < cin) return TP_ERR_INVALID;
  if (wd && (cout_p < cout || cin_p2 < cin)) return TP_ERR_INVALID;
  if (wf_ld <= 0) wf_ld = r * s * cin_p;
  if (wf_ld < r * s * cin_p) return TP_ERR_INVALID;
  cudaStream_t st = (cudaStream_t)stream;
  const int rs = r * s;
  int max_c = kSlabFloats / (kCoT * rs); if (max_c < 1) return TP_ERR_UNSUPPORTED;
  int ysplit = (cin + max_c - 1) / max_c;
  int cc = (cin + ysplit - 1) / ysplit;
  size_t smem = (size_t)kCoT * cc * rs * sizeof(float);
  if (wd) {
    long long nz = (long long)cin_p2 * rs * cout_p;
    if (cout_p > cout || cin_p2 > cin) {
      launch(k_zero_bf16, (unsigned)min((nz + 255) / 256, (long long)sm_count() * 16), 256, 0, st, (__nv_bfloat16*)wd, nz);
    }
  }
  const int kmf_words = (int)tp_kblock_mask_words(wf_ld), kmd_words = (int)tp_kblock_mask_words((int64_t)rs * cout_p);
  if (kmask_f) TP_CUDA_CHECK(cudaMemsetAsync(kmask_f, 0, ((size_t)((cout + 63) / 64) * kmf_words + 1) * 4, st));
  if (kmask_d && wd) TP_CUDA_CHECK(cudaMemsetAsync(kmask_d, 0, ((size_t)((cin + 63) / 64) * kmd_words + 1) * 4, st));
  dim3 grid((cout + kCoT - 1) / kCoT, ysplit);
  launch(k_stage_weights, grid, 256, smem, st, (const float*)w, (const float*)mask, cout, cin, rs,
                                           (__nv_bfloat16*)wf, cin_p, (__nv_bfloat16*)wd, cout_p, wf_ld,
                                           (uint32_t*)kmask_f, kmf_words, (uint32_t*)kmask_d, kmd_words);
  if (kmask_f || (kmask_d && wd))
    launch(k_kmask_summary1, 1, 256, 0, st, (uint32_t*)kmask_f, (cout + 63) / 64, kmf_words, (wf_ld + 63) / 64,
                                         wd ? (uint32_t*)kmask_d : nullptr, (cin + 63) / 64, kmd_words, (rs * cout_p + 63) / 64);
  TP_LAUNCH_CHECK();
  return TP_OK;
}

size_t tp_stage_batched_workspace_bytes(int n_items) {
  return n_items > 0 ? (size_t)n_items * sizeof(StageItem) + 512 : 0;
}

int tp_stage_weights_batched(const tp_stage_item* items, int n_items, int table_cached, void* kmask_all, size_t kmask_bytes,
                             void* ws, size_t ws_bytes, void* stream) {
  if (!items || n_items <= 0 || !ws) return TP_ERR_INVALID;
  cudaStream_t st = (cudaStream_t)stream;
  Arena ar(ws, ws_bytes);
  StageItem* d_items = (StageItem*)ar.take(sizeof(StageItem) * n_items);
  if (!d_items) return TP_ERR_WORKSPACE;
  std::vector<StageItem> h(n_items);
  long long cta = 0; size_t smem = 0;
  for (int i = 0; i < n_items; ++i) {
    const tp_stage_item& q = items[i];
    if (!q.w || !q.mask || !q.wf || q.cout <= 0 || q.cin <= 0 || q.r <= 0 || q.s <= 0 || q.cin_p < q.cin) return TP_ERR_INVALID;
    if (q.wd && q.cout_p < q.cout) return TP_ERR_INVALID;
    const int rs = q.r * q.s;
    int max_c = kSlabFloats / (kCoT * rs); if (max_c < 1) return TP_ERR_UNSUPPORTED;
    const int ysplit = (q.cin + max_c - 1) / max_c;
    const int cc = (q.cin + ysplit - 1) / ysplit;
    StageItem& t = h[i];
    t.w = (const float*)q.w; t.mask = (const float*)q.mask; t.wf = (__nv_bfloat16*)q.wf; t.wd = (__nv_bfloat16*)q.wd;
    t.cout = q.cout; t.cin = q.cin; t.rs = rs; t.cin_p = q.cin_p; t.cout_p = q.cout_p; t.ysplit = ysplit; t.cc = cc;
    t.wf_ld = q.wf_ld > 0 ? q.wf_ld : rs * q.cin_p;
    if (t.wf_ld < rs * q.cin_p) return TP_ERR_INVALID;
    t.cta0 = cta;
    t.kmf = (uint32_t*)q.kmask_f; t.kmd = (uint32_t*)q.kmask_d;
    t.kmf_words = (int)tp_kblock_mask_words(t.wf_ld); t.kmd_words = (int)tp_kblock_mask_words((int64_t)rs * q.cout_p);
    cta += (long long)((q.cout + kCoT - 1) / kCoT) * ysplit;
    const size_t need = (size_t)kCoT * cc * rs * sizeof(float);
    if (need > smem) smem = need;
  }
  if (cta > 0x7fffffffll) return TP_ERR_UNSUPPORTED;
  if (!table_cached)
    TP_CUDA_CHECK(cudaMemcpyAsync(d_items, h.data(), sizeof(StageItem) * n_items, cudaMemcpyHostToDevice, st));
  if (kmask_all && kmask_bytes) TP_CUDA_CHECK(cudaMemsetAsync(kmask_all, 0, kmask_bytes, st));
  launch(k_stage_weights_batched, (unsigned)cta, 256, smem, st, d_items, n_items);
  if (kmask_all && kmask_bytes) launch(k_kmask_summary, n_items, 256, 0, st, d_items, n_items);
  TP_LAUNCH_CHECK();
  return TP_OK;
}

int tp_to_nhwc_bf16(const void* src, int src_dtype, int64_t sn, int64_t sc, int64_t sh, int64_t sw,
                    int n, int c, int h, int w, void* dst, int c_pad, void* stream) {
  if (!src || !dst || n <= 0 || c <= 0 || h <= 0 || w <= 0 || c_pad < c) return TP_ERR_INVALID;
  cudaStream_t st = (cudaStream_t)stream;
  long long total = (long long)n * h * w * c_pad;
  unsigned grid = (unsigned)min((total + 255) / 256, (long long)sm_count() * 32);
  if (src_dtype == 0) launch(k_to_nhwc<float>, grid, 256, 0, st, (const float*)src, sn, sc, sh, sw, n, c, h, w, (__nv_bfloat16*)dst, c_pad);
  else if (src_dtype == 1) launch(k_to_nhwc<__nv_bfloat16>, grid, 256, 0, st, (const __nv_bfloat16*)src, sn, sc, sh, sw, n, c, h, w, (__nv_bfloat16*)dst, c_pad);
  else return TP_ERR_INVALID;
  TP_LAUNCH_CHECK();
  return TP_OK;
}

int tp_im2col_c8(const void* x, int n, int h, int w, int r, int s, int stride_h, int stride_w,
                 int pad_h, int pad_w, int p, int q, void* xcol, int kp, void* stream) {
  if (!x || !xcol || n <= 0 || kp % 8 != 0 || kp < r * s * 8) return TP_ERR_INVALID;
  cudaStream_t st = (cudaStream_t)stream;
  const long long total = (long long)n * p * q * (kp / 8);
  unsigned grid = (unsigned)min((total + 255) / 256, (long long)sm_count() * 32);
  launch(k_im2col_c8, grid, 256, 0, st, (const uint4*)x, n, h, w, r, s, stride_h, stride_w, pad_h, pad_w, p, q, (uint4*)xcol, kp / 8);
  TP_LAUNCH_CHECK();
  return TP_OK;
}

int tp_im2col_stem(const void* src, int src_dtype, int64_t sn, int64_t sc, int64_t sh, int64_t sw,
                   int n, int c, int h, int w, int r, int s, int cg, int stride_h, int stride_w, int pad_h, int pad_w,
                   int p, int q, void* xcol, int kp, void* stream) {
  if (!src || !xcol || n <= 0 || c <= 0 || c > 8 || cg < c || cg > 8 || kp % 8 != 0 || kp < r * s * cg) return TP_ERR_INVALID;
  if (r > 255 || s > 255 || kp > 8192) return TP_ERR_UNSUPPORTED;
  cudaStream_t st = (cudaStream_t)stream;
  {
    const int QS = q < 128 ? q : 128;
    const int pw = (QS - 1) * stride_w + s;
    const size_t patch = ((size_t)r * pw * c + 8) * sizeof(unsigned short);
    const char* e = getenv("TP_STEM_IM2COL");
    if (patch <= 40 * 1024 && kp / 8 <= 256 && !(e && e[0] == 'c')) {
      const long long strips = (long long)n * p * ((q + QS - 1) / QS);
      const unsigned g2 = (unsigned)min(strips, (long long)sm_count() * 8);
      if (src_dtype == 0)
        launch(k_im2col_stem_rows<float>, g2, 256, patch, st, (const float*)src, sn, sc, sh, sw, n, c, h, w, r, s, cg, stride_h, stride_w, pad_h, pad_w, p, q, QS, (uint4*)xcol, kp / 8);
      else if (src_dtype == 1)
        launch(k_im2col_stem_rows<__nv_bfloat16>, g2, 256, patch, st, (const __nv_bfloat16*)src, sn, sc, sh, sw, n, c, h, w, r, s, cg, stride_h, stride_w, pad_h, pad_w, p, q, QS, (uint4*)xcol, kp / 8);
      else return TP_ERR_INVALID;
      TP_LAUNCH_CHECK();
      return TP_OK;
    }
  }
  const long long total = (long long)n * p * q * (kp / 8);
  unsigned grid = (unsigned)min((total + 255) / 256, (long long)sm_count() * 32);
  const size_t smem = (size_t)kp * sizeof(uint32_t);
  if (src_dtype == 0)
    launch(k_im2col_stem<float>, grid, 256, smem, st, (const float*)src, sn, sc, sh, sw, n, c, h, w, r, s, cg, stride_h, stride_w, pad_h, pad_w, p, q, (uint4*)xcol, kp / 8);
  else if (src_dtype == 1)
    launch(k_im2col_stem<__nv_bfloat16>, grid, 256, smem, st, (const __nv_bfloat16*)src, sn, sc, sh, sw, n, c, h, w, r, s, cg, stride_h, stride_w, pad_h, pad_w, p, q, (uint4*)xcol, kp / 8);
  else return TP_ERR_INVALID;
  TP_LAUNCH_CHECK();
  return TP_OK;
}

int tp_sgd_momentum(void* const* w, const void* const* g, void* const* buf, const int64_t* numel,
                    int n_seg, const float* lr_dev, float momentum, float weight_decay,
                    int first_step, int table_cached, void* ws, size_t ws_bytes, void* stream) {
  if (!numel || n_seg <= 0 || !lr_dev || !ws) return TP_ERR_INVALID;
  if (!table_cached && (!w || !g || !buf)) return TP_ERR_INVALID;
  cudaStream_t st = (cudaStream_t)stream;
  Arena ar(ws, ws_bytes);
  Seg* d_segs = nullptr; long long tiles = 0;
  if (table_cached) {
    d_segs = (Seg*)ar.take(sizeof(Seg) * n_seg);
    if (!d_segs) return TP_ERR_WORKSPACE;
    for (int i = 0; i < n_seg; ++i) tiles += (numel[i] + kTileElems - 1) / kTileElems;
  } else {
    int rc = upload_segs(ar, (const void* const*)w, g, nullptr, nullptr, buf, numel, n_seg, &d_segs, &tiles, nullptr, st);
    if (rc) return rc;
  }
  if (tiles == 0) return TP_OK;
  long long gmax = (long long)sm_count() * 8;
  launch(k_sgd, (unsigned)(tiles < gmax ? tiles : gmax), 256, 0, st, d_segs, n_seg, tiles, lr_dev, momentum, weight_decay, first_step);
  TP_LAUNCH_CHECK();
  return TP_OK;
}

}
```

### turboprune_b200/ops.py

```python
import ctypes
from ctypes import c_void_p

import torch

from . import _cabi

_launches = 0


def _count(n=1):
    global _launches
    _launches += n


def launch_count() -> int:
    return _launches


class KernelTimer:

    def __init__(self):
        self.records = []

    def totals(self):
        out = {}
        for kind, flops, e0, e1 in self.records:
            ms = e0.elapsed_time(e1)
            t = out.setdefault(kind, [0.0, 0.0, 0])
            t[0] += ms; t[1] += flops; t[2] += 1
        return out


_timer = None


def set_timer(timer):
    global _timer
    _timer = timer


class _Timed:
    def __init__(self, kind, desc, cin_real=None):
        self.on = _timer is not None
        if self.on:
            cin = desc.cin if cin_real is None else cin_real
            self.flops = 2.0 * desc.n * desc.p * desc.q * desc.cout * cin * desc.r * desc.s
            self.kind = kind

    def __enter__(self):
        if self.on:
            self.e0 = torch.cuda.Event(enable_timing=True); self.e0.record()

    def __exit__(self, *a):
        if self.on:
            e1 = torch.cuda.Event(enable_timing=True); e1.record()
            _timer.records.append((self.kind, self.flops, self.e0, e1))


_grad_ready_hook = None


def set_grad_ready_hook(fn):
    global _grad_ready_hook
    _grad_ready_hook = fn


def get_grad_ready_hook():
    return _grad_ready_hook


def grad_ready(*slots):
    if _grad_ready_hook is not None:
        for s in slots:
            if s is not None:
                _grad_ready_hook(s.data_ptr())


WGRAD_SIDE_STREAM = False
_wgrad_streams = {}
_wgrad_keepalive = []


def set_wgrad_side_stream(on: bool):
    global WGRAD_SIDE_STREAM
    WGRAD_SIDE_STREAM = bool(on)


def _wgrad_stream(device):
    st = _wgrad_streams.get(device.index)
    if st is None:
        st = _wgrad_streams[device.index] = torch.cuda.Stream(device)
    return st


def join_wgrad(device=None):
    if not _wgrad_keepalive:
        return
    devs = {t[0].device for t in _wgrad_keepalive}
    for d in devs:
        if device is None or d == device:
            torch.cuda.current_stream(d).wait_stream(_wgrad_stream(d))
    _wgrad_keepalive.clear()


def _require_cuda(*tensors):
    for t in tensors:
        if t is not None and not t.is_cuda:
            raise RuntimeError("turboprune_b200 kernels need CUDA tensors (H100 / sm_90a); there is no CPU path")


_ws_cache = {}


def _workspace(nbytes: int, device, tag="default") -> torch.Tensor:
    key = (device.index, torch.cuda.current_stream(device).cuda_stream, tag)
    buf = _ws_cache.get(key)
    if buf is None or buf.numel() < nbytes:
        buf = torch.empty(max(int(nbytes), 1 << 16), dtype=torch.uint8, device=device)
        _ws_cache[key] = buf
    return buf


def topk_threshold_mask(ws, ms, k, gs=None, kind=_cabi.TP_SCORE_MAG, write_masks=True):
    lib = _cabi.load()
    _require_cuda(*ws, *ms)
    dev = ws[0].device
    ws = [w.detach().contiguous() for w in ws]
    ms = [m.detach().contiguous() for m in ms]
    gs = None if gs is None else [g.detach().contiguous() for g in gs]
    for t in ws + ms + (gs or []):
        if t.dtype != torch.float32:
            raise TypeError("pruning kernels operate on fp32 weights / masks / grads")
    numel = [w.numel() for w in ws]
    total = sum(numel)
    outs = [torch.empty_like(m) for m in ms] if write_masks else None
    thr = torch.empty((), dtype=torch.float32, device=dev)
    nbytes = lib.tp_topk_workspace_bytes(len(ws), total)
    wsb = _workspace(nbytes, dev, "topk")
    info = (ctypes.c_int64 * 4)()
    with torch.cuda.device(dev):
        rc = lib.tp_topk_threshold_mask(
            _cabi.ptr_array(ws), _cabi.ptr_array(gs), _cabi.ptr_array(ms), _cabi.ptr_array(outs),
            _cabi.i64_array(numel), len(ws), int(k), int(kind), c_void_p(thr.data_ptr()),
            c_void_p(wsb.data_ptr()), wsb.numel(), info, _cabi.stream_ptr(dev))
    if rc == _cabi.TP_ERR_K_RANGE:
        raise RuntimeError(f"kthvalue(): selected number k out of range for dimension 0 (k={k}, N={total})")
    _cabi.check(rc, "tp_topk_threshold_mask")
    _count(1)
    return outs, thr, {"path": int(info[0]), "candidates": int(info[1]), "n_lt": int(info[2]), "nan_thr": bool(info[3])}


class TopKPlan:

    def __init__(self, ws, ms, gs=None, kind=_cabi.TP_SCORE_MAG):
        self.lib = _cabi.load()
        self.dev = ws[0].device
        self.ws = [w.detach().contiguous() for w in ws]
        self.ms = [m.detach().contiguous() for m in ms]
        self.gs = None if gs is None else [g.detach().contiguous() for g in gs]
        self.outs = [torch.empty_like(m) for m in self.ms]
        self.thr = torch.empty((), dtype=torch.float32, device=self.dev)
        self.n = len(self.ws)
        self.total = sum(w.numel() for w in self.ws)
        self.kind = int(kind)
        self.wsb = torch.empty(self.lib.tp_topk_workspace_bytes(self.n, self.total), dtype=torch.uint8, device=self.dev)
        self.args = (_cabi.ptr_array(self.ws), _cabi.ptr_array(self.gs), _cabi.ptr_array(self.ms), _cabi.ptr_array(self.outs),
                     _cabi.i64_array([w.numel() for w in self.ws]))
        self.info = (ctypes.c_int64 * 4)()
        self._cached = False

    def enqueue(self, k):
        with torch.cuda.device(self.dev):
            rc = self.lib.tp_topk_enqueue(*self.args, self.n, int(k), self.kind, c_void_p(self.thr.data_ptr()),
                                          c_void_p(self.wsb.data_ptr()), self.wsb.numel(), int(self._cached),
                                          _cabi.stream_ptr(self.dev))
        if rc == _cabi.TP_ERR_K_RANGE:
            raise RuntimeError(f"kthvalue(): selected number k out of range for dimension 0 (k={k}, N={self.total})")
        _cabi.check(rc, "tp_topk_enqueue")
        self._cached = True
        _count(1)

    def finish(self, k):
        with torch.cuda.device(self.dev):
            rc = self.lib.tp_topk_finish(self.args[2], self.args[3], self.args[4], self.n, int(k), self.kind,
                                         c_void_p(self.thr.data_ptr()), c_void_p(self.wsb.data_ptr()), self.wsb.numel(),
                                         self.info, _cabi.stream_ptr(self.dev))
        _cabi.check(rc, "tp_topk_finish")
        return self.outs, self.thr, {"path": int(self.info[0]), "candidates": int(self.info[1]), "n_lt": int(self.info[2]),
                                     "nan_thr": bool(self.info[3])}

    def run(self, k):
        self.enqueue(k)
        return self.finish(k)


def apply_threshold(ws, ms, thr, gs=None, kind=_cabi.TP_SCORE_MAG):
    lib = _cabi.load()
    _require_cuda(*ws, *ms, thr)
    dev = ws[0].device
    ws = [w.detach().contiguous() for w in ws]
    ms = [m.detach().contiguous() for m in ms]
    gs = None if gs is None else [g.detach().contiguous() for g in gs]
    outs = [torch.empty_like(m) for m in ms]
    thr = thr.to(device=dev, dtype=torch.float32).reshape(())
    wsb = _workspace(lib.tp_segtable_workspace_bytes(len(ws)), dev, "seg")
    with torch.cuda.device(dev):
        rc = lib.tp_apply_threshold(_cabi.ptr_array(ws), _cabi.ptr_array(gs), _cabi.ptr_array(ms), _cabi.ptr_array(outs),
                                    _cabi.i64_array([w.numel() for w in ws]), len(ws), int(kind),
                                    c_void_p(thr.data_ptr()), c_void_p(wsb.data_ptr()), wsb.numel(), _cabi.stream_ptr(dev))
    _cabi.check(rc, "tp_apply_threshold")
    _count()
    return outs


def count_zeros(ms):
    lib = _cabi.load()
    _require_cuda(*ms)
    dev = ms[0].device
    ms = [m.detach().contiguous() for m in ms]
    out = torch.empty(len(ms) + 1, dtype=torch.int64, device=dev)
    wsb = _workspace(lib.tp_segtable_workspace_bytes(len(ms)), dev, "seg")
    with torch.cuda.device(dev):
        rc = lib.tp_count_zeros(_cabi.ptr_array(ms), _cabi.i64_array([m.numel() for m in ms]), len(ms),
                                c_void_p(out.data_ptr()), c_void_p(wsb.data_ptr()), wsb.numel(), _cabi.stream_ptr(dev))
    _cabi.check(rc, "tp_count_zeros")
    _count()
    return out


def sgd_momentum_step(params, grads, bufs, lr_dev, momentum, weight_decay, first_step, table_ws=None, table_cached=False):
    lib = _cabi.load()
    dev = params[0].device
    wsb = table_ws if table_ws is not None else _workspace(lib.tp_segtable_workspace_bytes(len(params)), dev, "seg")
    with torch.cuda.device(dev):
        rc = lib.tp_sgd_momentum(_cabi.ptr_array(params), _cabi.ptr_array(grads), _cabi.ptr_array(bufs),
                                 _cabi.i64_array([p.numel() for p in params]), len(params),
                                 c_void_p(lr_dev.data_ptr()), float(momentum), float(weight_decay), int(bool(first_step)),
                                 int(bool(table_cached)), c_void_p(wsb.data_ptr()), wsb.numel(), _cabi.stream_ptr(dev))
    _cabi.check(rc, "tp_sgd_momentum")
    _count()


def _round_up(x, m):
    return (x + m - 1) // m * m


def make_desc(n, h, w, cin, cout, r, s, stride, padding):
    sh, sw = stride
    ph, pw = padding
    p = (h + 2 * ph - r) // sh + 1
    q = (w + 2 * pw - s) // sw + 1
    return _cabi.ConvDesc(n, h, w, cin, cout, r, s, sh, sw, ph, pw, p, q)


def stem_geometry(cin, r, s):
    cg = cin
    return cg, _round_up(r * s * cg, 8)


KBLOCK_SKIP = True


def set_kblock_skip(on: bool):
    global KBLOCK_SKIP
    KBLOCK_SKIP = bool(on)


def kmask_shapes(cout, cin, r, s, wf_ld, cout_p):
    words = lambda cols: ((cols + 63) // 64 + 31) // 32
    return ((cout + 63) // 64, words(wf_ld)), ((cin + 63) // 64, words(r * s * cout_p))


def kblock_occupancy(kmask, columns):
    kb = (columns + 63) // 64
    rows = kmask_rows(kmask, columns)
    return int(kmask[-1].item()), rows.shape[0] * kb


def stage_weights(weight4d, mask4d, cin_p, need_dgrad, cout_p=None, wf_ld=0, want_kmask=None):
    lib = _cabi.load()
    cout, cin, r, s = weight4d.shape
    dev = weight4d.device
    if wf_ld and wf_ld > r * s * cin_p:
        wf = torch.zeros(cout, wf_ld, dtype=torch.bfloat16, device=dev)
    else:
        wf = torch.empty(cout, r * s * cin_p, dtype=torch.bfloat16, device=dev)
    wd = None
    cout_p = cout if cout_p is None else cout_p
    if need_dgrad:
        wd = torch.empty(cin, r * s * cout_p, dtype=torch.bfloat16, device=dev)
    kf = kd = None
    if KBLOCK_SKIP if want_kmask is None else want_kmask:
        sf, sd = kmask_shapes(cout, cin, r, s, wf.shape[1], cout_p)
        kf = torch.empty(sf[0] * sf[1] + 1, dtype=torch.int32, device=dev)
        kd = torch.empty(sd[0] * sd[1] + 1, dtype=torch.int32, device=dev) if wd is not None else None
    with torch.cuda.device(dev):
        rc = lib.tp_stage_weights(c_void_p(weight4d.data_ptr()), c_void_p(mask4d.data_ptr()), cout, cin, r, s,
                                  c_void_p(wf.data_ptr()), cin_p, int(wf_ld), c_void_p(wd.data_ptr()) if wd is not None else None,
                                  cout_p, cin, c_void_p(kf.data_ptr()) if kf is not None else None,
                                  c_void_p(kd.data_ptr()) if kd is not None else None, _cabi.stream_ptr(dev))
    _cabi.check(rc, "tp_stage_weights")
    _count()
    wf.kmask = kf
    if wd is not None:
        wd.kmask = kd
    return wf, wd


def kmask_rows(kmask, columns):
    words = ((columns + 63) // 64 + 31) // 32
    return kmask[:-1].view(-1, words)


def padded_cin(cin, r, s):
    return _round_up(cin, 64 if r * s > 1 else 8)


def _operand_plan(cout, cin, r, s):
    if cin <= 8 and (cin % 8 != 0 or r * s > 1):
        cg, kp = stem_geometry(cin, r, s)
        return cg, cout, False, kp
    cin_p = padded_cin(cin, r, s)
    return cin_p, _round_up(cout, 64 if r * s > 1 else 8), True, r * s * cin_p


class WeightStager:

    def __init__(self, layers):
        self.layers = [l for l in layers]
        self._key = None
        self._bufs = None
        self._items = None
        self._ws = None

    @staticmethod
    def _shape4(layer):
        w = layer.weight
        if w.dim() == 4:
            return tuple(w.shape)
        return (w.shape[0], w.shape[1], 1, 1)

    def _rebuild(self, key):
        dev = self.layers[0].weight.device
        if self._bufs is None:
            self._bufs = []
            for l in self.layers:
                cout, cin, r, s = self._shape4(l)
                plan = _operand_plan(cout, cin, r, s)
                if plan is None or not l.weight.is_cuda or l.weight.dtype != torch.float32 or not l.weight.is_contiguous():
                    self._bufs.append(None)
                    continue
                cin_p, cout_p, has_wd, wf_ld = plan
                wf = torch.zeros(cout, wf_ld, dtype=torch.bfloat16, device=dev)
                wd = torch.zeros(cin, r * s * cout_p, dtype=torch.bfloat16, device=dev) if has_wd else None
                self._bufs.append((wf, wd, cin_p, cout_p))
            shapes = []
            for l, b in zip(self.layers, self._bufs):
                if b is None:
                    shapes.append(None); continue
                cout, cin, r, s = self._shape4(l)
                shapes.append(kmask_shapes(cout, cin, r, s, b[0].shape[1], b[3]))
            total = sum(sf[0] * sf[1] + 1 + ((sd[0] * sd[1] + 1) if b[1] is not None else 0)
                        for (sh, b) in zip(shapes, self._bufs) if sh is not None for sf, sd in [sh])
            self._kmask_all = torch.zeros(max(total, 1), dtype=torch.int32, device=dev)
            off = 0
            for sh, b in zip(shapes, self._bufs):
                if sh is None:
                    continue
                sf, sd = sh
                b[0].kmask = self._kmask_all[off:off + sf[0] * sf[1] + 1]; off += sf[0] * sf[1] + 1
                if b[1] is not None:
                    b[1].kmask = self._kmask_all[off:off + sd[0] * sd[1] + 1]; off += sd[0] * sd[1] + 1
        live = [(l, b) for l, b in zip(self.layers, self._bufs) if b is not None]
        items = (_cabi.StageItem * len(live))()
        for it, (l, (wf, wd, cin_p, cout_p)) in zip(items, live):
            cout, cin, r, s = self._shape4(l)
            it.w = l.weight.data_ptr(); it.mask = l.mask.data_ptr()
            it.wf = wf.data_ptr(); it.wd = wd.data_ptr() if wd is not None else None
            it.cout, it.cin, it.r, it.s, it.cin_p, it.cout_p, it.wf_ld = cout, cin, r, s, cin_p, cout_p, wf.shape[1]
            it.kmask_f = wf.kmask.data_ptr()
            it.kmask_d = wd.kmask.data_ptr() if wd is not None else None
        self._items, self._live, self._key = items, live, key
        if self._ws is None:
            lib = _cabi.load()
            self._ws = torch.empty(max(int(lib.tp_stage_batched_workspace_bytes(len(self.layers))), 256), dtype=torch.uint8, device=dev)

    def stage(self):
        lib = _cabi.load()
        for l in self.layers:
            if l.mask.device != l.weight.device or l.mask.dtype != torch.float32 or not l.mask.is_contiguous():
                l.mask = l.mask.to(device=l.weight.device, dtype=torch.float32).contiguous()
        key = tuple((l.weight.data_ptr(), l.mask.data_ptr()) for l in self.layers)
        cached = key == self._key
        if not cached:
            self._rebuild(key)
        if not len(self._live):
            return
        dev = self.layers[0].weight.device
        with torch.cuda.device(dev):
            rc = lib.tp_stage_weights_batched(self._items, len(self._live), int(cached), c_void_p(self._kmask_all.data_ptr()),
                                              self._kmask_all.numel() * 4, c_void_p(self._ws.data_ptr()),
                                              self._ws.numel(), _cabi.stream_ptr(dev))
        _cabi.check(rc, "tp_stage_weights_batched")
        _count()
        for l, (wf, wd, _, _) in self._live:
            l.__dict__["_tp_staged"] = (wf, wd)


def skipped_block_report(stager):
    rows, empty, total = [], 0, 0
    for l, b in zip(stager.layers, stager._bufs):
        if b is None or getattr(b[0], "kmask", None) is None:
            continue
        e, t = kblock_occupancy(b[0].kmask, b[0].shape[1])
        rows.append((type(l).__name__, tuple(l.weight.shape), e, t))
        empty += e; total += t
    return {"empty_blocks": empty, "total_blocks": total, "fraction": empty / max(total, 1), "layers": rows}


def take_staged(layer):
    st = layer.__dict__.get("_tp_staged")
    if st is not None:
        layer.__dict__["_tp_staged"] = None
    return st


def to_nhwc_bf16(x, c_pad):
    lib = _cabi.load()
    n, c, h, w = x.shape
    if x.dtype == torch.bfloat16 and c == c_pad and x.permute(0, 2, 3, 1).is_contiguous():
        return x.permute(0, 2, 3, 1)
    if x.dtype not in (torch.float32, torch.bfloat16):
        x = x.float()
    out = torch.empty(n, h, w, c_pad, dtype=torch.bfloat16, device=x.device)
    sn, sc, sh, sw = x.stride()
    with torch.cuda.device(x.device):
        rc = lib.tp_to_nhwc_bf16(c_void_p(x.data_ptr()), 0 if x.dtype == torch.float32 else 1, sn, sc, sh, sw,
                                 n, c, h, w, c_void_p(out.data_ptr()), c_pad, _cabi.stream_ptr(x.device))
    _cabi.check(rc, "tp_to_nhwc_bf16")
    _count()
    return out


def im2col_c8(x_nhwc8, desc, kp):
    lib = _cabi.load()
    n, h, w, _ = x_nhwc8.shape
    out = torch.empty(n * desc.p * desc.q, kp, dtype=torch.bfloat16, device=x_nhwc8.device)
    with torch.cuda.device(x_nhwc8.device):
        rc = lib.tp_im2col_c8(c_void_p(x_nhwc8.data_ptr()), n, h, w, desc.r, desc.s, desc.stride_h, desc.stride_w,
                              desc.pad_h, desc.pad_w, desc.p, desc.q, c_void_p(out.data_ptr()), kp,
                              _cabi.stream_ptr(x_nhwc8.device))
    _cabi.check(rc, "tp_im2col_c8")
    _count()
    return out


def empty_cl(n, c, h, w, device):
    return torch.empty((n, c, h, w), dtype=torch.bfloat16, device=device, memory_format=torch.channels_last)


def im2col_stem(x, desc, kp, cg):
    lib = _cabi.load()
    n, c, h, w = x.shape
    if x.dtype not in (torch.float32, torch.bfloat16):
        x = x.float()
    out = torch.empty(n * desc.p * desc.q, kp, dtype=torch.bfloat16, device=x.device)
    sn, sc, sh, sw = x.stride()
    with torch.cuda.device(x.device):
        rc = lib.tp_im2col_stem(c_void_p(x.data_ptr()), 0 if x.dtype == torch.float32 else 1, sn, sc, sh, sw, n, c, h, w,
                                desc.r, desc.s, cg, desc.stride_h, desc.stride_w, desc.pad_h, desc.pad_w, desc.p, desc.q,
                                c_void_p(out.data_ptr()), kp, _cabi.stream_ptr(x.device))
    _cabi.check(rc, "tp_im2col_stem")
    _count()
    return out


def conv_fprop(desc, x_nhwc, wf, bias=None, out=None, want_stats=False):
    lib = _cabi.load()
    dev = x_nhwc.device
    y = out if out is not None else torch.empty(desc.n, desc.p, desc.q, desc.cout, dtype=torch.bfloat16, device=dev)
    stats = None
    if want_stats:
        stats = torch.empty(int(lib.tp_conv_stats_rows(ctypes.byref(desc))), 2, desc.cout, dtype=torch.float32, device=dev)
    with torch.cuda.device(dev), _Timed("fprop", desc):
        km = getattr(wf, "kmask", None) if KBLOCK_SKIP else None
        rc = lib.tp_conv_fprop_stats(ctypes.byref(desc), c_void_p(x_nhwc.data_ptr()), c_void_p(wf.data_ptr()),
                                     c_void_p(km.data_ptr()) if km is not None else None,
                                     c_void_p(bias.data_ptr()) if bias is not None else None, c_void_p(y.data_ptr()),
                                     c_void_p(stats.data_ptr()) if stats is not None else None,
                                     None, 0, _cabi.stream_ptr(dev))
    _cabi.check(rc, "tp_conv_fprop")
    _count()
    return (y, stats) if want_stats else y


def conv_dgrad(desc, dy_nhwc, wd, addend=None, kmask=None):
    lib = _cabi.load()
    dev = dy_nhwc.device
    dx = torch.empty(desc.n, desc.h, desc.w, desc.cin, dtype=torch.bfloat16, device=dev)
    with torch.cuda.device(dev), _Timed("dgrad", desc):
        km = (kmask if kmask is not None else getattr(wd, "kmask", None)) if KBLOCK_SKIP else None
        rc = lib.tp_conv_dgrad(ctypes.byref(desc), c_void_p(dy_nhwc.data_ptr()), c_void_p(wd.data_ptr()),
                               c_void_p(km.data_ptr()) if km is not None else None,
                               c_void_p(addend.data_ptr()) if addend is not None else None,
                               c_void_p(dx.data_ptr()), None, 0, _cabi.stream_ptr(dev))
    _cabi.check(rc, "tp_conv_dgrad")
    _count(1 if desc.stride_h == 1 and desc.stride_w == 1 else desc.stride_h * desc.stride_w)
    return dx


BN_BWD_FUSION = True


def set_bn_bwd_fusion(on: bool):
    global BN_BWD_FUSION
    BN_BWD_FUSION = bool(on)


def conv_dgrad_bnrelu(desc, dy_nhwc, wd, bn_src, kmask=None):
    lib = _cabi.load()
    dev = dy_nhwc.device
    y, weight, bias, mean, invstd = bn_src[:5]
    g = torch.empty(desc.n, desc.h, desc.w, desc.cin, dtype=torch.bfloat16, device=dev)
    rows = int(lib.tp_conv_dgrad_partial_rows(ctypes.byref(desc)))
    partial = torch.empty(rows, 2, desc.cin, dtype=torch.float32, device=dev)
    km = (kmask if kmask is not None else getattr(wd, "kmask", None)) if KBLOCK_SKIP else None
    P = lambda t: c_void_p(t.data_ptr()) if t is not None else None
    with torch.cuda.device(dev), _Timed("dgrad", desc):
        rc = lib.tp_conv_dgrad_bnrelu(ctypes.byref(desc), P(dy_nhwc), P(wd), P(km), P(y), P(weight), P(bias), P(mean), P(invstd),
                                      P(g), P(partial), _cabi.stream_ptr(dev))
    if rc == -5:
        return None
    _cabi.check(rc, "tp_conv_dgrad_bnrelu")
    _count()
    return g, partial


def conv_wgrad(desc, x_nhwc, dy_nhwc, mask4d, cin_real, want_db=False, dw_out=None, db_out=None, kmask=None):
    lib = _cabi.load()
    dev = x_nhwc.device
    dw = dw_out if dw_out is not None else torch.empty(desc.cout, cin_real, desc.r, desc.s, dtype=torch.float32, device=dev)
    db = (db_out if db_out is not None else torch.empty(desc.cout, dtype=torch.float32, device=dev)) if want_db else None
    nbytes = lib.tp_conv_workspace_bytes(ctypes.byref(desc), 2)
    wsb = _workspace(nbytes, dev, "wgrad")
    with torch.cuda.device(dev), _Timed("wgrad", desc):
        km = kmask if KBLOCK_SKIP else None
        rc = lib.tp_conv_wgrad(ctypes.byref(desc), c_void_p(x_nhwc.data_ptr()), c_void_p(dy_nhwc.data_ptr()),
                               c_void_p(mask4d.data_ptr()), c_void_p(km.data_ptr()) if km is not None else None,
                               cin_real, c_void_p(dw.data_ptr()),
                               c_void_p(db.data_ptr()) if db is not None else None,
                               c_void_p(wsb.data_ptr()), wsb.numel(), _cabi.stream_ptr(dev))
    _cabi.check(rc, "tp_conv_wgrad")
    _count(3 if want_db else 2)
    return dw, db


class MaskedConv2dFn(torch.autograd.Function):

    @staticmethod
    def forward(ctx, x, weight, mask, bias, stride, padding, want_skip=False, grad_slots=None, staged=None, want_stats=False,
                bn_src=None):
        _require_cuda(x, weight, mask)
        ctx.set_materialize_grads(False)
        ctx.bn_src = None
        ctx.want_skip = want_skip
        ctx.want_stats = want_stats
        stats = None
        ctx.grad_slots = grad_slots
        cout, cin, r, s = weight.shape
        n, _, h, w = x.shape
        need_dx = ctx.needs_input_grad[0]
        w32 = weight.detach().contiguous()
        m32 = mask.detach().contiguous()
        cin_p = padded_cin(cin, r, s)
        small_c = cin <= 8 and cin_p != cin and not need_dx
        desc = make_desc(n, h, w, cin_p if not small_c else cin, cout, r, s, stride, padding)
        cout_p = _round_up(cout, 64 if (r * s > 1 and not small_c) else 8)
        if small_c:
            cg, kp = stem_geometry(cin, r, s)
            xg = im2col_stem(x, desc, kp, cg)
            gdesc = _cabi.ConvDesc(n * desc.p * desc.q, 1, 1, kp, cout, 1, 1, 1, 1, 0, 0, 1, 1)
            if staged is not None and staged[0].shape == (cout, kp):
                wf, wd = staged
            else:
                wf, wd = stage_weights(w32, m32, cg, False, wf_ld=kp)
            y = empty_cl(n, cout, desc.p, desc.q, x.device)
            if want_stats:
                _, stats = conv_fprop(gdesc, xg, wf, bias, out=y, want_stats=True)
            else:
                conv_fprop(gdesc, xg, wf, bias, out=y)
            ctx.mode = "stem"
            ctx.gdesc = gdesc
            ctx.save_for_backward(xg, m32)
        else:
            xn = to_nhwc_bf16(x, cin_p)
            if (staged is not None and staged[0].shape == (cout, r * s * cin_p)
                    and (not need_dx or (staged[1] is not None and staged[1].shape == (cin, r * s * cout_p)))):
                wf, wd = staged
            else:
                wf, wd = stage_weights(w32, m32, cin_p, need_dx, cout_p)
            y = empty_cl(n, cout, desc.p, desc.q, x.device)
            if want_stats:
                _, stats = conv_fprop(desc, xn, wf, bias, out=y, want_stats=True)
            else:
                conv_fprop(desc, xn, wf, bias, out=y)
            ctx.mode = "conv"
            ctx.save_for_backward(xn, m32, wd)
            if (bn_src is not None and BN_BWD_FUSION and need_dx and not want_skip and stride == (1, 1) and cin_p == cin
                    and bn_src[0].shape == xn.shape):
                ctx.bn_src = bn_src
            ctx.wd_kmask = getattr(wd, "kmask", None) if wd is not None else None
            ctx.wf_kmask = getattr(wf, "kmask", None)
        ctx.desc = desc
        ctx.cin = cin
        ctx.has_bias = bias is not None
        ctx.cout_p = cout_p
        ctx.x_dtype = x.dtype
        if want_skip:
            if want_stats:
                ctx.mark_non_differentiable(stats)
                return y, x, stats
            return y, x
        if want_stats:
            ctx.mark_non_differentiable(stats)
            return y, stats
        return y

    @staticmethod
    def backward(ctx, dy, *rest):
        dskip = rest[0] if ctx.want_skip and rest else None
        desc = ctx.desc
        if dy is None:
            return dskip, None, None, None, None, None, None, None, None, None, None
        cout = desc.cout
        need_dx, need_dw = ctx.needs_input_grad[0], ctx.needs_input_grad[1]
        need_db = ctx.has_bias and ctx.needs_input_grad[3]
        dyn = to_nhwc_bf16(dy, ctx.cout_p)
        dx = dw = db = None
        db_in_slot = False
        if ctx.mode == "stem":
            xg, m32 = ctx.saved_tensors
            if need_dw:
                r, s = desc.r, desc.s
                cin = m32.shape[1]
                ones = torch.ones(cout, xg.shape[1], dtype=torch.float32, device=xg.device)
                gd = ctx.gdesc
                dwm, db = conv_wgrad(gd, xg, dyn.view(-1, cout), ones.view(cout, -1, 1, 1), xg.shape[1], need_db)
                cg = stem_geometry(cin, r, s)[0]
                dw = dwm[:, :r * s * cg].reshape(cout, r * s, cg)[:, :, :cin].permute(0, 2, 1).reshape(cout, cin, r, s) * m32
        else:
            xn, m32, wd = ctx.saved_tensors
            cin = ctx.cin
            ddesc = desc
            if ctx.cout_p != cout:
                ddesc = _cabi.ConvDesc(desc.n, desc.h, desc.w, desc.cin, ctx.cout_p, desc.r, desc.s, desc.stride_h,
                                       desc.stride_w, desc.pad_h, desc.pad_w, desc.p, desc.q)
            if need_dx:
                addend = None
                if dskip is not None:
                    addend = to_nhwc_bf16(dskip, cin)
                xdesc = ddesc if cin == desc.cin else _cabi.ConvDesc(desc.n, desc.h, desc.w, cin, ctx.cout_p, desc.r, desc.s,
                                                                      desc.stride_h, desc.stride_w, desc.pad_h, desc.pad_w,
                                                                      desc.p, desc.q)
                fused = None
                if ctx.bn_src is not None and addend is None:
                    fused = conv_dgrad_bnrelu(xdesc, dyn, wd, ctx.bn_src, kmask=ctx.wd_kmask)
                if fused is not None:
                    g, partial = fused
                    from . import fused_norm
                    fused_norm.offer_partials(g, partial, ctx.bn_src[5])
                    dx = g.permute(0, 3, 1, 2)
                else:
                    dx = conv_dgrad(xdesc, dyn, wd, addend, kmask=ctx.wd_kmask).permute(0, 3, 1, 2)
                if dx.dtype != ctx.x_dtype:
                    dx = dx.to(ctx.x_dtype)
            if need_dw:
                if ctx.cout_p != cout:
                    m_p = torch.zeros(ctx.cout_p, *m32.shape[1:], dtype=torch.float32, device=m32.device)
                    m_p[:cout] = m32
                    dwp, dbp = conv_wgrad(ddesc, xn, dyn, m_p, cin, need_db)
                    dw = dwp[:cout].contiguous()
                    db = dbp[:cout].contiguous() if dbp is not None else None
                else:
                    ws_, bs_ = ctx.grad_slots if ctx.grad_slots is not None else (None, None)
                    direct_w = ws_ is not None and ws_.is_contiguous() and ws_.numel() == m32.numel()
                    direct_b = need_db and bs_ is not None
                    if WGRAD_SIDE_STREAM and direct_w and (direct_b or not need_db):
                        dev = xn.device
                        cur, side = torch.cuda.current_stream(dev), _wgrad_stream(dev)
                        ev = torch.cuda.Event(); ev.record(cur)
                        side.wait_event(ev)
                        with torch.cuda.stream(side):
                            conv_wgrad(desc, xn, dyn, m32, cin, need_db, dw_out=ws_, db_out=bs_ if direct_b else None,
                                       kmask=ctx.wf_kmask)
                            grad_ready(ws_, bs_ if direct_b else None)
                        _wgrad_keepalive.append((xn, dyn, m32))
                        dw = db = None
                        db_in_slot = direct_b
                    else:
                        dw, db = conv_wgrad(desc, xn, dyn, m32, cin, need_db, dw_out=ws_ if direct_w else None,
                                            db_out=bs_ if direct_b else None, kmask=ctx.wf_kmask)
                        if direct_w:
                            dw = None
                        if direct_b:
                            db = None
                            db_in_slot = True
                        grad_ready(ws_ if direct_w else None, bs_ if direct_b else None)
        if need_db and db is None and not db_in_slot:
            db = dy.float().sum(dim=(0, 2, 3))
        if dskip is not None and dx is None and need_dx is False:
            dx = None
        return dx, dw, None, db, None, None, None, None, None, None, None


def masked_conv2d(x, weight, mask, bias=None, stride=(1, 1), padding=(0, 0), want_skip=False, grad_slots=None, staged=None,
                  want_stats=False, bn_src=None):
    return MaskedConv2dFn.apply(x, weight, mask, bias, tuple(stride), tuple(padding), want_skip, grad_slots, staged, want_stats,
                                bn_src)


def masked_linear(x, weight2d, mask2d, bias=None, grad_slots=None, staged=None):
    shp = x.shape
    x2 = x.reshape(-1, shp[-1])
    y = MaskedConv2dFn.apply(x2.view(x2.shape[0], x2.shape[1], 1, 1), weight2d.view(*weight2d.shape, 1, 1),
                             mask2d.view(*mask2d.shape, 1, 1), bias, (1, 1), (0, 0), False, grad_slots, staged)
    return y.reshape(*shp[:-1], weight2d.shape[0])
```

Measured before the change: 5711.

## Replace stem im2col with in-kernel gather fprop and space-to-depth wgrad

The 7x7 stride-2 stem conv no longer materializes a 147-column im2col buffer. The forward igemm gets a GATHER mode in which all 128 producer threads build A tiles directly from a padded NHWC input. Backward weight grad runs on a space-to-depth (16-channel, 4x1 tap) view through the existing wgrad path, and the finalize kernel remaps the result back to 7x7 taps. This cuts memory traffic and the large im2col buffer, at the cost of a new prep kernel, a different producer register split, and a more complex producer.

```diff
diff --git a/include/turboprune_b200.h b/include/turboprune_b200.h
--- a/include/turboprune_b200.h
+++ b/include/turboprune_b200.h
@@ -71,6 +71,9 @@
                    int n, int c, int h, int w, int r, int s, int cg, int stride_h, int stride_w, int pad_h, int pad_w,
                    int p, int q, void* xcol, int kp, void* stream);
 
+int tp_stem_s2d(const void* src, int src_dtype, int64_t sn, int64_t sc, int64_t sh, int64_t sw,
+                int n, int c, int h, int w, void* xs, void* xp, void* stream);
+
 int tp_cifar_augment(const void* src, void* out, const int64_t* idx, const int64_t* shifts, const uint8_t* flip,
                      const int64_t* cut_y, const int64_t* cut_x, int cut_size,
                      int n, int c, int h, int w, int r, void* stream);
@@ -108,6 +111,11 @@
                          void* g, void* partial, void* stream);
 int tp_conv_wgrad(const tp_conv_desc* d, const void* x, const void* dy, const void* mask, const void* kmask_f,
                   int cin_real, void* dw, void* db, void* ws, size_t ws_bytes, void* stream);
+
+int tp_conv_fprop_stem(const tp_conv_desc* d, const void* xp, const void* wf, const void* kmask_f, const void* bias_f32,
+                       void* y, void* stats, void* stream);
+int tp_conv_wgrad_s2d(const tp_conv_desc* d, const void* xs, const void* dy, const void* mask, void* dw, void* db,
+                      void* ws, size_t ws_bytes, void* stream);
 
 int tp_bn_forward_ext(const void* y, const void* residual, void* z, int64_t M, int C,
                       const void* weight, const void* bias, void* running_mean, void* running_var,
diff --git a/turboprune_b200/_cabi.py b/turboprune_b200/_cabi.py
--- a/turboprune_b200/_cabi.py
+++ b/turboprune_b200/_cabi.py
@@ -51,6 +51,8 @@
                                 c_void_p, c_int, c_void_p]),
     "tp_im2col_c8": (c_int, [c_void_p] + [c_int] * 11 + [c_void_p, c_int, c_void_p]),
     "tp_im2col_stem": (c_int, [c_void_p, c_int, c_int64, c_int64, c_int64, c_int64] + [c_int] * 13 + [c_void_p, c_int, c_void_p]),
+    "tp_stem_s2d": (c_int, [c_void_p, c_int, c_int64, c_int64, c_int64, c_int64, c_int, c_int, c_int, c_int, c_void_p, c_void_p,
+                            c_void_p]),
     "tp_cifar_augment": (c_int, [c_void_p, c_void_p, c_void_p, c_void_p, c_void_p, c_void_p, c_void_p, c_int, c_int, c_int, c_int, c_int, c_int, c_void_p]),
     "tp_resized_crop": (c_int, [c_void_p, c_int, c_int, POINTER(c_float), POINTER(c_float), c_void_p, c_void_p]),
     "tp_synth_normal": (c_int, [c_void_p, c_int64, c_uint64, c_uint64, c_int, c_void_p]),
@@ -59,6 +61,9 @@
     "tp_conv_fprop": (c_int, [POINTER(ConvDesc), c_void_p, c_void_p, c_void_p, c_void_p, c_void_p, c_size_t, c_void_p]),
     "tp_conv_stats_rows": (c_size_t, [POINTER(ConvDesc)]),
     "tp_conv_fprop_stats": (c_int, [POINTER(ConvDesc), c_void_p, c_void_p, c_void_p, c_void_p, c_void_p, c_void_p, c_void_p, c_size_t, c_void_p]),
+    "tp_conv_fprop_stem": (c_int, [POINTER(ConvDesc), c_void_p, c_void_p, c_void_p, c_void_p, c_void_p, c_void_p, c_void_p]),
+    "tp_conv_wgrad_s2d": (c_int, [POINTER(ConvDesc), c_void_p, c_void_p, c_void_p, c_void_p, c_void_p, c_void_p, c_size_t,
+                                  c_void_p]),
     "tp_conv_dgrad": (c_int, [POINTER(ConvDesc), c_void_p, c_void_p, c_void_p, c_void_p, c_void_p, c_void_p, c_size_t, c_void_p]),
     "tp_conv_dgrad_partial_rows": (c_size_t, [POINTER(ConvDesc)]),
     "tp_conv_dgrad_bnrelu": (c_int, [POINTER(ConvDesc), c_void_p, c_void_p, c_void_p, c_void_p, c_void_p, c_void_p, c_void_p, c_void_p,
diff --git a/turboprune_b200/csrc/tp_common.cuh b/turboprune_b200/csrc/tp_common.cuh
--- a/turboprune_b200/csrc/tp_common.cuh
+++ b/turboprune_b200/csrc/tp_common.cuh
@@ -87,6 +87,9 @@
   return lo;
 }
 
+constexpr int kS2dK = 7;
+constexpr int kS2dCh = 16;
+
 __device__ __forceinline__ float4 ld_stream(const float4* p) {
   float4 r;
   asm volatile("ld.global.nc.L1::no_allocate.v4.f32 {%0,%1,%2,%3}, [%4];"
diff --git a/turboprune_b200/csrc/tp_core.cu b/turboprune_b200/csrc/tp_core.cu
--- a/turboprune_b200/csrc/tp_core.cu
+++ b/turboprune_b200/csrc/tp_core.cu
@@ -98,7 +98,7 @@
 }
 
 const char* tp_last_cuda_error(void) { return tp::g_last_err; }
-int tp_abi_version(void) { return 10; }
+int tp_abi_version(void) { return 11; }
 int tp_device_sm_count(void) { return tp::sm_count(); }
 int tp_set_pdl(int on) { const int prev = tp::pdl_enabled() ? 1 : 0; tp::g_pdl = on ? 1 : 0; return prev; }
 
diff --git a/turboprune_b200/csrc/tp_igemm.cu b/turboprune_b200/csrc/tp_igemm.cu
--- a/turboprune_b200/csrc/tp_igemm.cu
+++ b/turboprune_b200/csrc/tp_igemm.cu
@@ -57,6 +57,8 @@
   const float* bn_weight; const float* bn_bias; const float* bn_mean; const float* bn_invstd;
   const uint32_t* kmask;
   int kmask_words;
+  const __nv_bfloat16* gsrc;
+  int g_hp, g_wp;
   TapEntry taps[kMaxTaps];
 };
 
@@ -154,12 +156,47 @@
   }
 }
 
-template <int BLOCK_N, bool MULTI, bool BNB>
+template <int KB>
+__device__ __forceinline__ void stem_gather_block(uint32_t row_addr, int row, const __nv_bfloat16* src, long long rs, bool valid) {
+  constexpr int kReal = 147, kRun = 21, kWords = 11;
+  constexpr int c0 = KB * 64, r0 = c0 / kRun, r1 = ((c0 + 63 < kReal ? c0 + 63 : kReal - 1)) / kRun;
+  uint32_t wv[r1 - r0 + 1][kWords];
+#pragma unroll
+  for (int r = 0; r <= r1 - r0; ++r) {
+    const uint32_t* w32 = reinterpret_cast<const uint32_t*>(src + (r0 + r) * rs);
+#pragma unroll
+    for (int k = 0; k < kWords; ++k) wv[r][k] = valid ? __ldg(w32 + k) : 0u;
+  }
+  auto half = [&](int col) -> uint32_t {
+    if (col >= kReal) return 0u;
+    const uint32_t w = wv[col / kRun - r0][(col % kRun) >> 1];
+    return (col % kRun) & 1 ? w >> 16 : w & 0xffffu;
+  };
+#pragma unroll
+  for (int j = 0; j < 8; ++j) {
+    uint32_t v[4];
+#pragma unroll
+    for (int e = 0; e < 4; ++e) {
+      const int col = c0 + j * 8 + 2 * e, i = col % kRun;
+      if (col + 1 < kReal && (col + 1) / kRun == col / kRun)
+        v[e] = (i & 1) ? __byte_perm(wv[col / kRun - r0][i >> 1], wv[col / kRun - r0][(i >> 1) + 1], 0x5432)
+                       : wv[col / kRun - r0][i >> 1];
+      else
+        v[e] = half(col) | (half(col + 1) << 16);
+    }
+    sts128(row_addr + (uint32_t)((j ^ (row & 7)) << 4), make_uint4(v[0], v[1], v[2], v[3]));
+  }
+}
+
+template <int BLOCK_N, bool MULTI, bool BNB, bool GATHER = false>
 __global__ void __launch_bounds__(kFwdThreads, 1)
 k_igemm_fwd(const __grid_constant__ AMaps tmA, const __grid_constant__ CUtensorMap tmB,
             const __grid_constant__ FwdParams p) {
   static_assert(BLOCK_N == 64 || BLOCK_N == 128, "wgmma N of the fwd kernel");
   static_assert(!BNB || !MULTI, "BatchNorm-backward epilogue: single class");
+  static_assert(!GATHER || (!MULTI && !BNB && BLOCK_N == 64), "stem gather: single class, forward epilogue, 64 channels");
+  constexpr int kProdRegs = GATHER ? 104 : kFwdProducerRegs, kConsRegs = GATHER ? 200 : kFwdConsumerRegs;
+  static_assert(kProdRegs * 128 + kConsRegs * 256 <= 168 * kFwdThreads, "fwd register split");
   constexpr int kABytes = kBlockM * kBlockK * 2;
   constexpr int kBBytes = BLOCK_N * kBlockK * 2;
   constexpr int kStageBytes = kABytes + kBBytes;
@@ -187,9 +224,9 @@
   };
 
   if (threadIdx.x == 0) {
-    for (int j = 0; j < p.ncls; ++j) prefetch_tmap(&tmA.m[j]);
+    if (!GATHER) for (int j = 0; j < p.ncls; ++j) prefetch_tmap(&tmA.m[j]);
     prefetch_tmap(&tmB);
-    for (int i = 0; i < kStages; ++i) { mbar_init(&full_bar[i], 1); mbar_init(&empty_bar[i], 1); }
+    for (int i = 0; i < kStages; ++i) { mbar_init(&full_bar[i], GATHER ? 129 : 1); mbar_init(&empty_bar[i], 1); }
     mbar_init(&order_bar[0], 1); mbar_init(&order_bar[1], 1);
     fence_mbar_init();
   }
@@ -197,8 +234,39 @@
   pdl_wait();
 
   if (warp < 4) {
-    setmaxnreg_dec<kFwdProducerRegs>();
-    if (threadIdx.x == 0) {
+    setmaxnreg_dec<kProdRegs>();
+    if (GATHER) {
+      const int row = threadIdx.x;
+      const uint32_t* const km = live_kmask(p.kmask, p.kmask_words, p.N);
+      const long long rs = (long long)p.g_wp * 3;
+      int stage = 0; uint32_t phase = 0;
+      for (int w = 0; w < my_items; ++w) {
+        int ci, m_g, n_t; get_tile(w, ci, m_g, n_t);
+        const int m = m_g * kBlockM + row;
+        const bool valid = m < p.M;
+        int n_, pp, qq; decompose_pixel(valid ? m : 0, p.cls[0].P_it, p.cls[0].Q_it, n_, pp, qq);
+        const __nv_bfloat16* src = p.gsrc + (((long long)n_ * p.g_hp + 2 * pp) * p.g_wp + 2 * qq) * 3;
+        KSkip ks; bool any = false;
+        if (km) ks.begin(km, p.kmask_words, n_t * BLOCK_N, BLOCK_N, p.N);
+        for (int kb = 0; kb < p.cchunks; ++kb) {
+          if (km && !ks.take(kb, kb == p.cchunks - 1, any)) continue;
+          any = true;
+          mbar_wait(&empty_bar[stage], phase ^ 1);
+          uint8_t* sA = smem + stage * kStageBytes;
+          if (row == 0) {
+            mbar_arrive_expect_tx(&full_bar[stage], kBBytes);
+            tma_load_2d(sA + kABytes, &tmB, &full_bar[stage], kb * kBlockK, n_t * BLOCK_N);
+          }
+          const uint32_t ra = smem_u32(sA) + (uint32_t)(row * 128);
+          if (kb == 0) stem_gather_block<0>(ra, row, src, rs, valid);
+          else if (kb == 1) stem_gather_block<1>(ra, row, src, rs, valid);
+          else stem_gather_block<2>(ra, row, src, rs, valid);
+          fence_proxy_async();
+          mbar_arrive(&full_bar[stage]);
+          if (++stage == kStages) { stage = 0; phase ^= 1; }
+        }
+      }
+    } else if (threadIdx.x == 0) {
       int stage = 0; uint32_t phase = 0;
       const uint32_t* const km = live_kmask(p.kmask, p.kmask_words, p.N);
       for (int w = 0; w < my_items; ++w) {
@@ -243,7 +311,7 @@
       }
     }
   } else {
-    setmaxnreg_inc<kFwdConsumerRegs>();
+    setmaxnreg_inc<kConsRegs>();
     const int cw = (warp >> 2) - 1;
     const int q = warp & 3;
     const int wtid = threadIdx.x & 127;
@@ -646,7 +714,7 @@
 __global__ void __launch_bounds__(256) k_wgrad_finalize(const float* __restrict__ partial, const float* __restrict__ mask,
                                                         float* __restrict__ dw, int cout, int cin_real, int cin_p, int rs,
                                                         int nb, int m_tiles, int splits, int sl,
-                                                        const uint32_t* __restrict__ kmask, int kmask_words) {
+                                                        const uint32_t* __restrict__ kmask, int kmask_words, int s2d_c) {
   pdl_enter();
   __shared__ float s_lane[256];
   const uint32_t* const km = live_kmask(kmask, kmask_words, cout);
@@ -682,10 +750,19 @@
   if (sj == 0 && kk < ktot) {
     float acc = 0.f;
     for (int j = 0; j < sl; ++j) acc += s_lane[j * KT + kl];
-    const int tap = kk / cin_p, ci = kk - tap * cin_p;
-    if (ci < cin_real) {
-      const long long o = ((long long)co * cin_real + ci) * rs + tap;
-      dw[o] = skipped ? 0.f : mask[o] * acc;
+    if (s2d_c) {
+      const int r = kk >> 6, s_ = (kk >> 4) & 3, g = (kk & 15) / s2d_c, ch = (kk & 15) - g * s2d_c;
+      const int kh = 2 * r - 1 + (g >> 1), kw = 2 * s_ - 1 + (g & 1);
+      if (g < 4 && kh >= 0 && kw >= 0) {
+        const long long o = (((long long)co * s2d_c + ch) * kS2dK + kh) * kS2dK + kw;
+        dw[o] = mask[o] * acc;
+      }
+    } else {
+      const int tap = kk / cin_p, ci = kk - tap * cin_p;
+      if (ci < cin_real) {
+        const long long o = ((long long)co * cin_real + ci) * rs + tap;
+        dw[o] = skipped ? 0.f : mask[o] * acc;
+      }
     }
   }
 }
@@ -797,9 +874,11 @@
 }
 
 static int make_im2col_map(CUtensorMap* m, const void* ptr, int n, int h, int w, int c,
-                           int base_w, int base_h, int step_w, int step_h, int P_it, int Q_it, uint32_t pixels) {
+                           int base_w, int base_h, int step_w, int step_h, int P_it, int Q_it, uint32_t pixels,
+                           int pix_c = 0, int row_pix = 0) {
+  const cuuint64_t pc = (cuuint64_t)(pix_c ? pix_c : c), rp = (cuuint64_t)(row_pix ? row_pix : w);
   cuuint64_t dims[4] = {(cuuint64_t)c, (cuuint64_t)w, (cuuint64_t)h, (cuuint64_t)n};
-  cuuint64_t strides[3] = {(cuuint64_t)c * 2, (cuuint64_t)w * c * 2, (cuuint64_t)h * w * c * 2};
+  cuuint64_t strides[3] = {pc * 2, rp * pc * 2, (cuuint64_t)h * rp * pc * 2};
   int lower[2] = {base_w, base_h};
   int upper[2] = {(Q_it - 1) * step_w + 1 + base_w - w, (P_it - 1) * step_h + 1 + base_h - h};
   cuuint32_t es[4] = {1, (cuuint32_t)step_w, (cuuint32_t)step_h, 1};
@@ -807,7 +886,7 @@
                               64, pixels, es, CU_TENSOR_MAP_INTERLEAVE_NONE, CU_TENSOR_MAP_SWIZZLE_128B,
                               CU_TENSOR_MAP_L2_PROMOTION_L2_256B, CU_TENSOR_MAP_FLOAT_OOB_FILL_NONE);
   if (r != CUDA_SUCCESS) return fail_cu(r, "cuTensorMapEncodeIm2col");
-  if (g_driver_version <= 13010 && (size_t)n * h * w * c * 2 < 131072)
+  if (g_driver_version <= 13010 && (size_t)n * strides[2] < 131072)
     reinterpret_cast<uint64_t*>(m)[1] &= ~(1ull << 21);
   return TP_OK;
 }
@@ -875,16 +954,28 @@
   return best;
 }
 
+constexpr int kStemCols = 152;
+
+static bool s2d_view(const tp_conv_desc* d, tp_conv_desc* v) {
+  if (!d || d->cin != 3 || d->r != kS2dK || d->s != kS2dK || d->stride_h != 2 || d->stride_w != 2 ||
+      d->pad_h != 3 || d->pad_w != 3 || d->n <= 0 || d->h <= 0 || d->w <= 0 || d->p != (d->h - 1) / 2 + 1 || d->q != (d->w - 1) / 2 + 1)
+    return false;
+  *v = *d;
+  v->h = d->p + 3; v->w = d->q; v->cin = 4 * kS2dCh; v->r = 4; v->s = 1;
+  v->stride_h = 1; v->stride_w = 1; v->pad_h = 0; v->pad_w = 0;
+  return true;
+}
+
 constexpr int kSmemMax = 232448;
 
-template <int BN, bool MULTI, bool BNB = false>
+template <int BN, bool MULTI, bool BNB = false, bool GATHER = false>
 static int launch_fwd(const AMaps& a, const CUtensorMap& b, FwdParams& p, cudaStream_t st) {
   constexpr int smem = fwd_smem(BN);
   static_assert(smem <= kSmemMax, "fwd smem budget");
   const int n_tiles = (p.N + BN - 1) / BN;
   static bool attr_set = false;
   if (!attr_set) {
-    TP_CUDA_CHECK(cudaFuncSetAttribute(k_igemm_fwd<BN, MULTI, BNB>, cudaFuncAttributeMaxDynamicSharedMemorySize, smem));
+    TP_CUDA_CHECK(cudaFuncSetAttribute(k_igemm_fwd<BN, MULTI, BNB, GATHER>, cudaFuncAttributeMaxDynamicSharedMemorySize, smem));
     attr_set = true;
   }
   long long ctiles = 0;
@@ -896,7 +987,7 @@
   }
   if (ctiles > 0x7fffffffll || ctiles <= 0) return TP_ERR_UNSUPPORTED;
   const int grid = (int)(ctiles < sm_count() ? ctiles : sm_count());
-  TP_CUDA_CHECK(launch(k_igemm_fwd<BN, MULTI, BNB>, dim3(grid), dim3(kFwdThreads), (size_t)smem, st, a, b, p));
+  TP_CUDA_CHECK(launch(k_igemm_fwd<BN, MULTI, BNB, GATHER>, dim3(grid), dim3(kFwdThreads), (size_t)smem, st, a, b, p));
   TP_LAUNCH_CHECK();
   return TP_OK;
 }
@@ -907,6 +998,11 @@
   p.staged_store = (p.ldc % 8 == 0 && p.N % 8 == 0 && (((uintptr_t)p.out) & 15) == 0 &&
                     (!p.addend || (((uintptr_t)p.addend) & 15) == 0)) ? 1 : 0;
   if (p.stats && !(p.staged_store && p.linear)) return TP_ERR_UNSUPPORTED;
+  if (p.gsrc) {
+    if (!p.linear) return TP_ERR_UNSUPPORTED;
+    if (bn != 64) return TP_ERR_UNSUPPORTED;
+    return launch_fwd<64, false, false, true>(a, b, p, st);
+  }
   const bool multi = !p.linear;
   if (multi) {
     if (bn == 128) return launch_fwd<128, true>(a, b, p, st);
@@ -942,6 +1038,12 @@
 
 size_t tp_conv_workspace_bytes(const tp_conv_desc* d, int op) {
   if (!d) return 0;
+  if (op == 3) {
+    tp_conv_desc v;
+    if (!s2d_view(d, &v)) return 0;
+    const WgGeom g = wgrad_geom(&v);
+    return g.partial_bytes(g.smax) + 1024;
+  }
   if (op != 2) return 256;
   const WgGeom g = wgrad_geom(d);
   return g.partial_bytes(g.smax) + 1024;
@@ -956,6 +1058,34 @@
 int tp_conv_fprop(const tp_conv_desc* d, const void* x, const void* wf, const void* bias_f32,
                   void* y, void* ws, size_t ws_bytes, void* stream) {
   return tp_conv_fprop_stats(d, x, wf, nullptr, bias_f32, y, nullptr, ws, ws_bytes, stream);
+}
+
+int tp_conv_fprop_stem(const tp_conv_desc* d, const void* xp, const void* wf, const void* kmask_f, const void* bias_f32,
+                       void* y, void* stats, void* stream) {
+  tp_conv_desc v;
+  if (!s2d_view(d, &v) || !xp || !wf || !y || (((uintptr_t)xp) & 3) != 0) return TP_ERR_INVALID;
+  if (stats && (d->cout % 8 != 0 || (((uintptr_t)y) & 15) != 0 || (((uintptr_t)stats) & 15) != 0)) return TP_ERR_UNSUPPORTED;
+  int rc = load_driver_fns(); if (rc) return rc;
+  rc = bind_device_of(xp); if (rc) return rc;
+  const int kp = kStemCols;
+  FwdParams p = {};
+  p.M = d->n * d->p * d->q; p.N = d->cout;
+  p.ncls = 1;
+  ClsEntry& ce = p.cls[0];
+  ce.M = p.M; ce.P_it = d->p; ce.Q_it = d->q; ce.ntaps = 1; ce.tap0 = 0; ce.oah = 0; ce.oaw = 0;
+  p.cchunks = (kp + 63) / 64;
+  p.out_img_pix = (long long)d->p * d->q; p.out_row_pix = d->q;
+  p.osh = 1; p.osw = 1;
+  p.ldc = d->cout; p.out = (__nv_bfloat16*)y; p.bias = (const float*)bias_f32;
+  p.stats = (float*)stats;
+  p.kmask = (const uint32_t*)kmask_f; p.kmask_words = (int)tp_kblock_mask_words(kp);
+  p.gsrc = (const __nv_bfloat16*)xp; p.g_hp = 2 * d->p + 5; p.g_wp = 2 * d->q + 6;
+  fill_taps(p.taps, 1, 1, kp);
+  AMaps ta = {};
+  CUtensorMap tb;
+  const int bn = pick_block_n((p.M + kBlockM - 1) / kBlockM, p.N);
+  rc = make_tiled_map(&tb, wf, (uint64_t)kp, (uint64_t)d->cout, (uint64_t)kp, (uint32_t)bn); if (rc) return rc;
+  return run_fwd(ta, tb, p, bn, (cudaStream_t)stream);
 }
 
 int tp_conv_fprop_stats(const tp_conv_desc* d, const void* x, const void* wf, const void* kmask_f, const void* bias_f32,
@@ -1105,8 +1235,24 @@
   return run_fwd(ta, tb, p, bn, st);
 }
 
+static int conv_wgrad_impl(const tp_conv_desc* d, const void* x, const void* dy, const void* mask, const void* kmask_f,
+                           int cin_real, void* dw, void* db, void* ws, size_t ws_bytes, void* stream, int s2d_c);
+
 int tp_conv_wgrad(const tp_conv_desc* d, const void* x, const void* dy, const void* mask, const void* kmask_f,
                   int cin_real, void* dw, void* db, void* ws, size_t ws_bytes, void* stream) {
+  return conv_wgrad_impl(d, x, dy, mask, kmask_f, cin_real, dw, db, ws, ws_bytes, stream, 0);
+}
+
+int tp_conv_wgrad_s2d(const tp_conv_desc* d, const void* xs, const void* dy, const void* mask, void* dw, void* db,
+                      void* ws, size_t ws_bytes, void* stream) {
+  tp_conv_desc v;
+  if (!s2d_view(d, &v)) return TP_ERR_INVALID;
+  if ((((uintptr_t)xs) & 15) != 0) return TP_ERR_INVALID;
+  return conv_wgrad_impl(&v, xs, dy, mask, nullptr, v.cin, dw, db, ws, ws_bytes, stream, d->cin);
+}
+
+static int conv_wgrad_impl(const tp_conv_desc* d, const void* x, const void* dy, const void* mask, const void* kmask_f,
+                           int cin_real, void* dw, void* db, void* ws, size_t ws_bytes, void* stream, int s2d_c) {
   if (!d || !x || !dy || !mask || !dw || !ws) return TP_ERR_INVALID;
   if (d->cin % 8 != 0 || d->cout % 8 != 0 || d->r * d->s > kMaxTaps || cin_real > d->cin) return TP_ERR_UNSUPPORTED;
   if (d->r * d->s > 1 && d->cin % 64 != 0) return TP_ERR_UNSUPPORTED;
@@ -1126,7 +1272,8 @@
   p.n_tiles = g.n_tiles;
   p.kblocks = g.kblocks;
   const int sms = sm_count();
-  int splits = pick_wgrad_splits(g);
+  tp_conv_desc gd = {d->n * d->p * d->q, 1, 1, kStemCols, d->cout, 1, 1, 1, 1, 0, 0, 1, 1};
+  int splits = pick_wgrad_splits(s2d_c ? wgrad_geom(&gd) : g);
   p.kb_per_split = (p.kblocks + splits - 1) / splits;
   splits = (p.kblocks + p.kb_per_split - 1) / p.kb_per_split;
   p.splits = splits;
@@ -1142,7 +1289,8 @@
   } else {
     p.b_mode = 1;
     p.base_w = -d->pad_w; p.base_h = -d->pad_h; p.step_w = d->stride_w; p.step_h = d->stride_h;
-    rc = make_im2col_map(&tb, x, d->n, d->h, d->w, d->cin, p.base_w, p.base_h, p.step_w, p.step_h, d->p, d->q, 64);
+    rc = make_im2col_map(&tb, x, d->n, d->h, d->w, d->cin, p.base_w, p.base_h, p.step_w, p.step_h, d->p, d->q, 64,
+                         s2d_c ? kS2dCh : 0, s2d_c ? d->q + 3 : 0);
     if (rc) return rc;
   }
   const int items = p.m_tiles * p.n_tiles * splits;
@@ -1158,7 +1306,7 @@
   const int fin_kt = 256 / sl;
   launch(k_wgrad_finalize, dim3(d->cout, (rs * d->cin + fin_kt - 1) / fin_kt), 256, 0, st,
       p.partial, (const float*)mask, (float*)dw, d->cout, cin_real, d->cin, rs, p.nb, p.m_tiles, splits, sl,
-      p.kmask, p.kmask_words);
+      p.kmask, p.kmask_words, s2d_c);
   TP_LAUNCH_CHECK();
   if (db) {
     const int c = d->cout, cv = c / 8;
diff --git a/turboprune_b200/csrc/tp_optim.cu b/turboprune_b200/csrc/tp_optim.cu
--- a/turboprune_b200/csrc/tp_optim.cu
+++ b/turboprune_b200/csrc/tp_optim.cu
@@ -308,6 +308,71 @@
       }
     }
   }
+}
+
+template <typename T, int C>
+__global__ void __launch_bounds__(256) k_stem_s2d(const T* __restrict__ src, long long sn, long long sc, long long sh, long long sw,
+                                                  int n, int h, int w, int hs, int ws, uint4* __restrict__ xs,
+                                                  __nv_bfloat16* __restrict__ xp) {
+  pdl_enter();
+  const long long total = (long long)n * hs * ws;
+  const long long step = (long long)gridDim.x * blockDim.x;
+  const int hp = 2 * hs - 1, wp = 2 * ws;
+  for (long long i = blockIdx.x * (long long)blockDim.x + threadIdx.x; i < total; i += step) {
+    const int j = (int)(i % ws); const long long t = i / ws;
+    const int ii = (int)(t % hs); const int ni = (int)(t / hs);
+    const T* base = src + ni * sn;
+    float f[kS2dCh];
+#pragma unroll
+    for (int k = 0; k < kS2dCh; ++k) f[k] = 0.f;
+#pragma unroll
+    for (int g = 0; g < 4; ++g) {
+      const int hh = 2 * ii - 4 + (g >> 1), ww = 2 * j - 4 + (g & 1);
+      if (hh < 0 || hh >= h || ww < 0 || ww >= w) continue;
+      const T* px = base + hh * sh + ww * sw;
+#pragma unroll
+      for (int ch = 0; ch < C; ++ch) f[g * C + ch] = (float)px[ch * sc];
+    }
+    uint32_t v[8];
+#pragma unroll
+    for (int k = 0; k < 8; ++k) {
+      const __nv_bfloat162 b = __floats2bfloat162_rn(f[2 * k], f[2 * k + 1]);
+      v[k] = *reinterpret_cast<const uint32_t*>(&b);
+    }
+    xs[2 * i] = make_uint4(v[0], v[1], v[2], v[3]);
+    xs[2 * i + 1] = make_uint4(v[4], v[5], v[6], v[7]);
+    if (xp) {
+#pragma unroll
+      for (int g = 0; g < 4; ++g) {
+        const int ph = 2 * ii - 1 + (g >> 1), pw = 2 * j - 1 + (g & 1);
+        if (ph < 0 || pw < 0) continue;
+        __nv_bfloat16* d = xp + (((long long)ni * hp + ph) * wp + pw) * C;
+#pragma unroll
+        for (int ch = 0; ch < C; ++ch) d[ch] = __float2bfloat16_rn(f[g * C + ch]);
+        if (pw == wp - 2)
+#pragma unroll
+          for (int ch = 0; ch < C; ++ch) d[C + ch] = __float2bfloat16_rn(0.f);
+      }
+    }
+  }
+}
+
+template <typename T>
+static int launch_stem_s2d(const void* src, int64_t sn, int64_t sc, int64_t sh, int64_t sw, int n, int c, int h, int w,
+                           int hs, int ws, void* xs, void* xp, cudaStream_t st) {
+  const long long total = (long long)n * hs * ws;
+  const unsigned grid = (unsigned)min((total + 255) / 256, (long long)sm_count() * 32);
+  const T* x = (const T*)src;
+  uint4* o = (uint4*)xs;
+  __nv_bfloat16* op = (__nv_bfloat16*)xp;
+  switch (c) {
+    case 1: launch(k_stem_s2d<T, 1>, grid, 256, 0, st, x, sn, sc, sh, sw, n, h, w, hs, ws, o, op); break;
+    case 2: launch(k_stem_s2d<T, 2>, grid, 256, 0, st, x, sn, sc, sh, sw, n, h, w, hs, ws, o, op); break;
+    case 3: launch(k_stem_s2d<T, 3>, grid, 256, 0, st, x, sn, sc, sh, sw, n, h, w, hs, ws, o, op); break;
+    default: launch(k_stem_s2d<T, 4>, grid, 256, 0, st, x, sn, sc, sh, sw, n, h, w, hs, ws, o, op); break;
+  }
+  TP_LAUNCH_CHECK();
+  return TP_OK;
 }
 
 __global__ void __launch_bounds__(256) k_sgd(const Seg* __restrict__ segs, int n_seg, long long tiles,
@@ -498,6 +563,17 @@
   return TP_OK;
 }
 
+int tp_stem_s2d(const void* src, int src_dtype, int64_t sn, int64_t sc, int64_t sh, int64_t sw,
+                int n, int c, int h, int w, void* xs, void* xp, void* stream) {
+  if (!src || !xs || n <= 0 || c <= 0 || c > 4 || h <= 0 || w <= 0) return TP_ERR_INVALID;
+  if ((((uintptr_t)xs) & 15) != 0) return TP_ERR_INVALID;
+  const int hs = (h - 1) / 2 + 1 + 3, ws = (w - 1) / 2 + 1 + 3;
+  cudaStream_t st = (cudaStream_t)stream;
+  if (src_dtype == 0) return launch_stem_s2d<float>(src, sn, sc, sh, sw, n, c, h, w, hs, ws, xs, xp, st);
+  if (src_dtype == 1) return launch_stem_s2d<__nv_bfloat16>(src, sn, sc, sh, sw, n, c, h, w, hs, ws, xs, xp, st);
+  return TP_ERR_INVALID;
+}
+
 int tp_sgd_momentum(void* const* w, const void* const* g, void* const* buf, const int64_t* numel,
                     int n_seg, const float* lr_dev, float momentum, float weight_decay,
                     int first_step, int table_cached, void* ws, size_t ws_bytes, void* stream) {
diff --git a/turboprune_b200/ops.py b/turboprune_b200/ops.py
--- a/turboprune_b200/ops.py
+++ b/turboprune_b200/ops.py
@@ -256,6 +256,18 @@
 def stem_geometry(cin, r, s):
     cg = cin
     return cg, _round_up(r * s * cg, 8)
+
+
+STEM_S2D = True
+
+
+def set_stem_s2d(on: bool):
+    global STEM_S2D
+    STEM_S2D = bool(on)
+
+
+def stem_s2d_applies(cin, r, s, stride, padding):
+    return STEM_S2D and cin == 3 and (r, s) == (7, 7) and tuple(stride) == (2, 2) and tuple(padding) == (3, 3)
 
 
 KBLOCK_SKIP = True
@@ -475,6 +487,58 @@
     return out
 
 
+def stem_s2d(x, want_padded=True):
+    lib = _cabi.load()
+    n, c, h, w = x.shape
+    if x.dtype not in (torch.float32, torch.bfloat16):
+        x = x.float()
+    P, Q = (h - 1) // 2 + 1, (w - 1) // 2 + 1
+    xs = torch.empty(n, P + 3, Q + 3, 16, dtype=torch.bfloat16, device=x.device)
+    xp = torch.empty(n, 2 * P + 5, 2 * Q + 6, c, dtype=torch.bfloat16, device=x.device) if want_padded else None
+    sn, sc, sh, sw = x.stride()
+    with torch.cuda.device(x.device):
+        rc = lib.tp_stem_s2d(c_void_p(x.data_ptr()), 0 if x.dtype == torch.float32 else 1, sn, sc, sh, sw, n, c, h, w,
+                             c_void_p(xs.data_ptr()), c_void_p(xp.data_ptr()) if xp is not None else None,
+                             _cabi.stream_ptr(x.device))
+    _cabi.check(rc, "tp_stem_s2d")
+    _count()
+    return xs, xp
+
+
+def conv_fprop_stem(desc, xp, wf, bias=None, out=None, want_stats=False):
+    lib = _cabi.load()
+    dev = xp.device
+    y = out if out is not None else torch.empty(desc.n, desc.p, desc.q, desc.cout, dtype=torch.bfloat16, device=dev)
+    stats = None
+    if want_stats:
+        stats = torch.empty(int(lib.tp_conv_stats_rows(ctypes.byref(desc))), 2, desc.cout, dtype=torch.float32, device=dev)
+    km = getattr(wf, "kmask", None) if KBLOCK_SKIP else None
+    with torch.cuda.device(dev), _Timed("fprop", desc):
+        rc = lib.tp_conv_fprop_stem(ctypes.byref(desc), c_void_p(xp.data_ptr()), c_void_p(wf.data_ptr()),
+                                    c_void_p(km.data_ptr()) if km is not None else None,
+                                    c_void_p(bias.data_ptr()) if bias is not None else None, c_void_p(y.data_ptr()),
+                                    c_void_p(stats.data_ptr()) if stats is not None else None, _cabi.stream_ptr(dev))
+    _cabi.check(rc, "tp_conv_fprop_stem")
+    _count()
+    return (y, stats) if want_stats else y
+
+
+def conv_wgrad_s2d(desc, xs, dy_nhwc, mask4d, want_db=False):
+    lib = _cabi.load()
+    dev = xs.device
+    dw = torch.empty(desc.cout, desc.cin, desc.r, desc.s, dtype=torch.float32, device=dev)
+    db = torch.empty(desc.cout, dtype=torch.float32, device=dev) if want_db else None
+    wsb = _workspace(lib.tp_conv_workspace_bytes(ctypes.byref(desc), 3), dev, "wgrad")
+    with torch.cuda.device(dev), _Timed("wgrad", desc):
+        rc = lib.tp_conv_wgrad_s2d(ctypes.byref(desc), c_void_p(xs.data_ptr()), c_void_p(dy_nhwc.data_ptr()),
+                                   c_void_p(mask4d.data_ptr()), c_void_p(dw.data_ptr()),
+                                   c_void_p(db.data_ptr()) if db is not None else None,
+                                   c_void_p(wsb.data_ptr()), wsb.numel(), _cabi.stream_ptr(dev))
+    _cabi.check(rc, "tp_conv_wgrad_s2d")
+    _count(3 if want_db else 2)
+    return dw, db
+
+
 def conv_fprop(desc, x_nhwc, wf, bias=None, out=None, want_stats=False):
     lib = _cabi.load()
     dev = x_nhwc.device
@@ -576,7 +640,22 @@
         small_c = cin <= 8 and cin_p != cin and not need_dx
         desc = make_desc(n, h, w, cin_p if not small_c else cin, cout, r, s, stride, padding)
         cout_p = _round_up(cout, 64 if (r * s > 1 and not small_c) else 8)
-        if small_c:
+        if small_c and stem_s2d_applies(cin, r, s, stride, padding):
+            cg, kp = stem_geometry(cin, r, s)
+            if staged is not None and staged[0].shape == (cout, kp):
+                wf = staged[0]
+            else:
+                wf, _ = stage_weights(w32, m32, cg, False, wf_ld=kp)
+            xs, xp = stem_s2d(x)
+            y = empty_cl(n, cout, desc.p, desc.q, x.device)
+            if want_stats:
+                _, stats = conv_fprop_stem(desc, xp, wf, bias, out=y, want_stats=True)
+            else:
+                conv_fprop_stem(desc, xp, wf, bias, out=y)
+            del xp
+            ctx.mode = "stem_s2d"
+            ctx.save_for_backward(xs, m32)
+        elif small_c:
             cg, kp = stem_geometry(cin, r, s)
             xg = im2col_stem(x, desc, kp, cg)
             gdesc = _cabi.ConvDesc(n * desc.p * desc.q, 1, 1, kp, cout, 1, 1, 1, 1, 0, 0, 1, 1)
@@ -638,7 +717,11 @@
         dyn = to_nhwc_bf16(dy, ctx.cout_p)
         dx = dw = db = None
         db_in_slot = False
-        if ctx.mode == "stem":
+        if ctx.mode == "stem_s2d":
+            xs, m32 = ctx.saved_tensors
+            if need_dw:
+                dw, db = conv_wgrad_s2d(desc, xs, dyn, m32, need_db)
+        elif ctx.mode == "stem":
             xg, m32 = ctx.saved_tensors
             if need_dw:
                 r, s = desc.r, desc.s
```

After: 5814 (median of 6 runs). 1.02x the previous value.
